# control-toolbox/CTDirect.jl

Hardware: AMD Instinct MI355X
Metric: NLP callback evals/s (constraints+sparse Jac), N-step Goddard, 1/2/4/8 GPU (higher is better)
Workload: dtype f64

## Files before the change

### ctdirect.jl_amd/_lib.py

```python
import ctypes as C
import os
import subprocess

_HERE = os.path.dirname(os.path.abspath(__file__))
LIB_PATH = os.environ.get("CTD_LIB_PATH") or os.path.join(_HERE, "libctdirect_hip.so")
CSRC = os.path.join(_HERE, "csrc")

CTD_OK, CTD_EINVAL, CTD_EGRID, CTD_ESCHEME, CTD_EPATTERN, CTD_EPROBLEM, CTD_ENODEVICE, CTD_EHIP, CTD_ENOMEM, CTD_ERCCL = range(10)


class ctd_desc(C.Structure):
    _fields_ = [("problem", C.c_int32), ("scheme", C.c_int32), ("pattern_mode", C.c_int32), ("device", C.c_int32),
                ("grid_size", C.c_int64), ("time_grid", C.POINTER(C.c_double)), ("time_grid_len", C.c_int64),
                ("step_begin", C.c_int64), ("step_end", C.c_int64), ("stream", C.c_void_p),
                ("stream_mode", C.c_int32), ("control_steps", C.c_int32), ("value_order", C.c_int32), ("reserved0", C.c_int32)]


class ctd_init(C.Structure):
    _fields_ = [("use_problem_default", C.c_int32), ("state", C.POINTER(C.c_double)),
                ("control", C.POINTER(C.c_double)), ("variable", C.POINTER(C.c_double)),
                ("n_samples", C.c_int64), ("t_samples", C.POINTER(C.c_double)),
                ("state_samples", C.POINTER(C.c_double)), ("control_samples", C.POINTER(C.c_double))]


class ctd_ocp_def(C.Structure):
    _fields_ = [("name", C.c_char_p), ("n", C.c_int32), ("m", C.c_int32), ("nv", C.c_int32), ("npath", C.c_int32),
                ("nbc", C.c_int32), ("it0", C.c_int32), ("itf", C.c_int32), ("t0", C.c_double), ("tf", C.c_double),
                ("maximize", C.c_int32), ("reserved", C.c_int32), ("dynamics", C.POINTER(C.c_char_p)),
                ("lagrange", C.c_char_p), ("mayer", C.c_char_p), ("path", C.POINTER(C.c_char_p)),
                ("boundary", C.POINTER(C.c_char_p)), ("constants", C.c_char_p)] + \
               [(k, C.POINTER(C.c_double)) for k in ("state_lb", "state_ub", "control_lb", "control_ub", "variable_lb",
                                                     "variable_ub", "path_lb", "path_ub", "boundary_lb", "boundary_ub")]


_dp = C.POINTER(C.c_double)
_ip = C.POINTER(C.c_int64)
_vp = C.c_void_p
SYMBOLS = {
    "ctd_create": (C.c_int32, [C.POINTER(ctd_desc), C.POINTER(_vp)]),
    "ctd_destroy": (C.c_int32, [_vp]),
    "ctd_last_error": (C.c_char_p, [_vp]),
    "ctd_strerror": (C.c_char_p, [C.c_int32]),
    "ctd_host_alloc": (C.c_int32, [C.POINTER(C.c_void_p), C.c_size_t]),
    "ctd_host_free": (C.c_int32, [C.c_void_p]),
    "ctd_sizes": (C.c_int32, [_vp, _ip, _ip, _ip, _ip]),
    "ctd_dims": (C.c_int32, [_vp, _ip]),
    "ctd_time_grid": (C.c_int32, [_vp, _dp, _dp]),
    "ctd_time_grid_at": (C.c_int32, [_vp, _dp, _dp]),
    "ctd_butcher": (C.c_int32, [_vp, _dp, _dp, _dp]),
    "ctd_bounds": (C.c_int32, [_vp, _dp, _dp, _dp, _dp]),
    "ctd_initial_guess": (C.c_int32, [_vp, _dp, C.POINTER(ctd_init)]),
    "ctd_jac_structure": (C.c_int32, [_vp, _ip, _ip]),
    "ctd_jac_csc": (C.c_int32, [_vp, _ip, _ip]),
    "ctd_jac_csr": (C.c_int32, [_vp, _ip, _ip]),
    "ctd_value_order": (C.c_int32, [_vp, C.POINTER(C.c_int32)]),
    "ctd_dropped_nonzeros": (C.c_int32, [_vp, _ip]),
    "ctd_obj": (C.c_int32, [_vp, _dp, _dp]),
    "ctd_grad": (C.c_int32, [_vp, _dp, _dp]),
    "ctd_grad_dev": (C.c_int32, [_vp, _vp, _vp]),
    "ctd_cons": (C.c_int32, [_vp, _dp, _dp]),
    "ctd_jac_coord": (C.c_int32, [_vp, _dp, _dp]),
    "ctd_cons_jac": (C.c_int32, [_vp, _dp, _dp, _dp]),
    "ctd_cons_jac_dev": (C.c_int32, [_vp, _vp, _vp, _vp]),
    "ctd_cons_jac_dev_async": (C.c_int32, [_vp, _vp, _vp, _vp]),
    "ctd_obj_dev": (C.c_int32, [_vp, _vp, _dp]),
    "ctd_obj_dev_async": (C.c_int32, [_vp, _vp, _vp]),
    "ctd_grad_dev_async": (C.c_int32, [_vp, _vp, _vp]),
    "ctd_grad_shard_dev_async": (C.c_int32, [_vp, _vp, _vp]),
    "ctd_sync": (C.c_int32, [_vp]),
    "ctd_set_stream": (C.c_int32, [_vp, _vp]),
    "ctd_shard_info": (C.c_int32, [_vp, _ip]),
    "ctd_time_cons_jac_dev": (C.c_int32, [_vp, _vp, _vp, _vp, C.c_int32, _dp]),
    "ctd_launch_info": (C.c_int32, [_vp, _ip]),
    "ctd_debug_stamps": (C.c_int32, [_vp, _vp, _vp, _vp, C.POINTER(C.c_uint64), C.c_int64]),
    "ctd_register_ocp": (C.c_int32, [C.POINTER(ctd_ocp_def), C.POINTER(C.c_int32)]),
    "ctd_ocp_source": (C.c_int32, [C.c_int32, C.c_char_p, C.c_int64]),
    "ctd_jit_check": (C.c_int32, [C.c_int32, C.c_int32]),
    "ctd_hess_structure": (C.c_int32, [_vp, _ip, _ip]),
    "ctd_hess_csc": (C.c_int32, [_vp, _ip, _ip]),
    "ctd_hess_csr": (C.c_int32, [_vp, _ip, _ip]),
    "ctd_hess_coord": (C.c_int32, [_vp, _dp, _dp, C.c_double, _dp]),
    "ctd_hess_coord_dev": (C.c_int32, [_vp, _vp, _vp, C.c_double, _vp]),
    "ctd_hess_coord_dev_async": (C.c_int32, [_vp, _vp, _vp, C.c_double, _vp]),
    "ctd_time_hess_dev": (C.c_int32, [_vp, _vp, _vp, C.c_double, _vp, C.c_int32, _dp]),
    "ctd_hess_launch_info": (C.c_int32, [_vp, _ip]),
    "ctd_hess_kernel_info": (C.c_int32, [_vp, _ip]),
    "ctd_hess_shard_info": (C.c_int32, [_vp, _ip]),
    "ctd_hess_debug_stamps": (C.c_int32, [_vp, _vp, _vp, C.c_double, _vp, C.POINTER(C.c_uint64), C.c_int64]),
    "ctd_eval_all_dev_async": (C.c_int32, [_vp, _vp, _vp, C.c_double, _vp, _vp, _vp, _vp, _vp]),
    "ctd_cons_jac_batch_dev_async": (C.c_int32, [_vp, C.c_int32, _vp, C.c_int64, _vp, C.c_int64, _vp, C.c_int64]),
    "ctd_obj_batch_dev_async": (C.c_int32, [_vp, C.c_int32, _vp, C.c_int64, _vp]),
    "ctd_grad_batch_dev_async": (C.c_int32, [_vp, C.c_int32, _vp, C.c_int64, _vp, C.c_int64]),
    "ctd_jprod": (C.c_int32, [_vp, _dp, _dp, _dp]),
    "ctd_jtprod": (C.c_int32, [_vp, _dp, _dp, _dp]),
    "ctd_jprod_dev_async": (C.c_int32, [_vp, _vp, _vp, _vp]),
    "ctd_jtprod_dev_async": (C.c_int32, [_vp, _vp, _vp, _vp]),
    "ctd_hprod": (C.c_int32, [_vp, _dp, _dp, C.c_double, _dp, _dp]),
    "ctd_hprod_dev_async": (C.c_int32, [_vp, _vp, _vp, C.c_double, _vp, _vp]),
    "ctd_kktprod": (C.c_int32, [_vp, _dp, _dp, C.c_double, _dp, _dp, _dp, _dp, _dp, _dp]),
    "ctd_kktprod_dev_async": (C.c_int32, [_vp, _vp, _vp, C.c_double, _vp, _vp, _vp, _vp, _vp, _vp]),
    "ctd_hdiag": (C.c_int32, [_vp, _dp, _dp, C.c_double, _dp]),
    "ctd_hdiag_dev_async": (C.c_int32, [_vp, _vp, _vp, C.c_double, _vp]),
    "ctd_jsq_rows": (C.c_int32, [_vp, _dp, _dp, _dp]),
    "ctd_jsq_rows_dev_async": (C.c_int32, [_vp, _vp, _vp, _vp]),
    "ctd_jsq_cols": (C.c_int32, [_vp, _dp, _dp, _dp]),
    "ctd_jsq_cols_dev_async": (C.c_int32, [_vp, _vp, _vp, _vp]),
    "ctd_jprod_shard_dev_async": (C.c_int32, [_vp, _vp, _vp, _vp]),
    "ctd_jtprod_shard_dev_async": (C.c_int32, [_vp, _vp, _vp, _vp]),
    "ctd_hprod_shard_dev_async": (C.c_int32, [_vp, _vp, _vp, C.c_double, _vp, _vp]),
    "ctd_kktprod_shard_dev_async": (C.c_int32, [_vp, _vp, _vp, C.c_double, _vp, _vp, _vp, _vp, _vp, _vp]),
    "ctd_hess_coord_batch_dev_async": (C.c_int32, [_vp, C.c_int32, _vp, C.c_int64, _vp, C.c_int64, C.c_double, _vp, C.c_int64]),
    "ctd_create_sharded": (C.c_int32, [C.POINTER(ctd_desc), C.POINTER(C.c_int32), C.c_int32, C.POINTER(_vp)]),
    "ctd_sharded_destroy": (C.c_int32, [_vp]),
    "ctd_sharded_last_error": (C.c_char_p, [_vp]),
    "ctd_sharded_handle": (C.c_int32, [_vp, C.c_int32, C.POINTER(_vp)]),
    "ctd_sharded_shard_info": (C.c_int32, [_vp, C.c_int32, _ip]),
    "ctd_cons_jac_sharded_dev_async": (C.c_int32, [_vp, C.POINTER(_vp), C.POINTER(_vp), C.POINTER(_vp), C.c_int32, C.c_int32]),
    "ctd_sharded_sync": (C.c_int32, [_vp]),
    "ctd_dev_alloc": (C.c_int32, [C.c_int32, C.c_size_t, C.POINTER(_vp)]),
    "ctd_dev_free": (C.c_int32, [C.c_int32, _vp]),
    "ctd_dev_copy": (C.c_int32, [C.c_int32, _vp, _vp, C.c_size_t, C.c_int32]),
    "ctd_set_x_shards": (C.c_int32, [_vp, C.c_int32, _ip, C.POINTER(_vp), C.c_int32]),
    "ctd_ipc_export": (C.c_int32, [C.c_int32, _vp, _vp, _ip]),
    "ctd_ipc_open": (C.c_int32, [C.c_int32, _vp, C.POINTER(_vp)]),
    "ctd_ipc_close": (C.c_int32, [C.c_int32, _vp]),
    "ctd_ipc_probe": (C.c_int32, [C.c_int32, _vp, C.c_size_t]),
    "ctd_stitch_c": (C.c_int32, [_vp, _vp, C.c_int32, C.c_int32, _vp]),
    "ctd_shard_steps": (C.c_int32, [C.c_int64, C.c_int32, C.c_int32, _ip, _ip]),
}


def build(jobs=8):
    subprocess.check_call(["make", "-C", CSRC, "-s", f"-j{jobs}"])
    return LIB_PATH


_lib = None


def lib():
    global _lib
    if _lib is None:
        if not os.path.exists(LIB_PATH):
            raise ImportError(
                f"{LIB_PATH} is missing: the HIP extension has not been built (run `python -c 'import "
                "__graft_entry__ as g; g.build()'` or `make -C ctdirect.jl_amd/csrc`). There is no fallback path.")
        try:
# ... 13 lines not shown
```

### ctdirect.jl_amd/csrc/ctd_engine.hip

```cpp
#include <hip/hip_runtime.h>
#include <hip/hiprtc.h>
#include <dlfcn.h>

#include <cstdio>
#include <functional>
#include <map>
#include <mutex>
#include <cstdlib>
#include <cstring>
#include <memory>
#include <new>
#include <string>
#include <vector>

#include "../../include/ctdirect_hip.h"
#include "ctd_host.hpp"
#include "ctd_kernels.hpp"
#include "ctd_hess_kernels.hpp"
#include "ctd_hess_step.hpp"
#include "ctd_iter_kernels.hpp"
#include "ctd_prod_kernels.hpp"
#include "ctd_hprod_kernels.hpp"
#include "ctd_kkt_kernels.hpp"
#include "ctd_diag_kernels.hpp"
#include "ctd_jit.hpp"

using namespace ctd;

namespace ctd {
#define CTD_EXTERN_ALL(ID, P) \
    CTD_EXTERN_LAUNCHERS(P) CTD_EXTERN_HESS(P) CTD_EXTERN_HESS_STEP(P) CTD_EXTERN_ITER(P) CTD_EXTERN_PROD(P) CTD_EXTERN_HPROD(P) CTD_EXTERN_KKT(P) CTD_EXTERN_DIAG(P)
CTD_REGISTRY(CTD_EXTERN_ALL)
}

template <class T = double> struct DevBuf {
    T* p = nullptr;
    int64_t cap = 0;
    DevBuf() = default;
    DevBuf(const DevBuf&) = delete;
    DevBuf& operator=(const DevBuf&) = delete;
    ~DevBuf() { release(); }
    void release() { if (p) (void)hipFree(p); p = nullptr; cap = 0; }
    hipError_t ensure(int64_t n) {
        if (p && n <= cap) return hipSuccess;
        release();
        const hipError_t e = hipMalloc((void**)&p, sizeof(T) * (size_t)(n > 1 ? n : 1));
        if (e == hipSuccess) cap = n; else p = nullptr;
        return e;
    }
    int32_t grow(ctd_handle* h, int64_t need, const char* fn);
};

enum JitFamily { JIT_FIRST, JIT_BATCH, JIT_PROD, JIT_HPROD, JIT_HESS, JIT_PROD_SHARD, JIT_HPROD_SHARD, JIT_KKT, JIT_KKT_SHARD, JIT_DIAG, kJitFamilies };
struct JitModule {
    hipModule_t mod = nullptr;
    hipFunction_t f[5] = {};
};

struct ctd_handle {
    Model model;
    int device = -1;
    hipStream_t stream = nullptr;
    bool own_stream = false;
    int64_t step_begin = 0, step_end = 0;
    int tile = 0, block = 256;
    int lean_ok = 1;
    KParams kp;
    size_t lds_bytes = 0;
    int grid = 0;
    DevBuf<double> d_tau;
    DevBuf<uint32_t> d_tmpl, d_vtmpl;
    DevBuf<uint16_t> d_pos;
    DevBuf<int64_t> d_edge_idx;
    DevBuf<uint32_t> d_edge_code;
    DevBuf<> d_x, d_c, d_vals;
    DevBuf<> d_partial;
    DevBuf<> d_obj;
    DevBuf<> d_g;
    DevBuf<> d_gpartial;
    int obj_blocks = 0;
    hipEvent_t ev0 = nullptr, ev1 = nullptr;
    const RtOcp* rt = nullptr;
    JitModule jit[kJitFamilies];
    bool hess_ready = false;
    HParams hp;
    int hess_tile = 0;
    size_t hess_lds_bytes = 0;
    DevBuf<uint32_t> d_htptr, d_hterms, d_hvptr, d_hvterms, d_heptr, d_hevptr, d_heterms;
    DevBuf<int64_t> d_hedge_idx;
    DevBuf<double> d_hpair_c;
    DevBuf<uint32_t> d_hcpos, d_hzpos;
    DevBuf<int32_t> d_hssrc, d_hschunk;
    DevBuf<double> d_hsck;
    bool hess_step = false;
    SParams sp{};
    HParams hp_step{};
    size_t hess_step_lds = 0;
    DevBuf<uint32_t> d_htasks, d_hptasks, d_hbtasks;
    DevBuf<> d_hpartials, d_y, d_hvals;
    DevBuf<XHalo> d_halo;
    XHalo halo_host{};
    DevBuf<> d_stitch_send, d_stitch_recv;
    int64_t hpart_member = 0;
    double out_mb = 0.0;
    DevBuf<> d_ppartial, d_pdir, d_pout;
    DevBuf<> d_hppartial;
    DevBuf<> d_kktpartial, d_kdy, d_ksx, d_ksc, d_krc;
    DevBuf<> d_hdpartial, d_jcpartial;
    std::string err;
};

constexpr double kWtMB = 64.0;
constexpr double kHessWtMB = 16.0;

static thread_local std::string g_create_err;

static int32_t fail(ctd_handle* h, int32_t code, const std::string& msg) {
    if (h) h->err = msg; else g_create_err = msg;
    return code;
}

#define HIP_TRY(h, expr)                                                                          \
    do {                                                                                          \
        hipError_t e_ = (expr);                                                                   \
        if (e_ != hipSuccess)                                                                     \
            return fail(h, CTD_EHIP, std::string(#expr) + ": " + hipGetErrorString(e_));          \
    } while (0)

struct DeviceGuard {
    int prev = -1;
    bool switched = false;
    hipError_t err = hipSuccess;
    DeviceGuard() = default;
    explicit DeviceGuard(int dev) { (void)bind(dev); }
    hipError_t bind(int dev) {
        err = hipGetDevice(&prev);
        if (err == hipSuccess && prev != dev) { err = hipSetDevice(dev); switched = (err == hipSuccess); }
        return err;
    }
    ~DeviceGuard() { if (switched) (void)hipSetDevice(prev); }
    DeviceGuard(const DeviceGuard&) = delete;
    DeviceGuard& operator=(const DeviceGuard&) = delete;
};

struct OnDevice {
    DeviceGuard dg;
    int32_t st = CTD_OK;
    explicit OnDevice(ctd_handle* h, const char* fn = nullptr) {
        if (!h) st = CTD_EINVAL;
        else if (h->device < 0)
            st = fail(h, CTD_ENODEVICE, std::string(fn ? fn : "") + (fn ? ": " : "") +
                                            "compute call on a host-only handle (device = -1); there is no CPU fallback");
        else if (dg.bind(h->device) != hipSuccess) st = fail(h, CTD_EHIP, std::string("dg_.err: ") + hipGetErrorString(dg.err));
    }
};

template <class T> int32_t DevBuf<T>::grow(ctd_handle* h, int64_t need, const char* fn) {
    if (need <= cap && p) return CTD_OK;
    hipStreamCaptureStatus cs = hipStreamCaptureStatusNone;
    if (hipStreamIsCapturing(h->stream, &cs) == hipSuccess && cs != hipStreamCaptureStatusNone)
        return fail(h, CTD_EINVAL, std::string(fn) + ": this batch needs larger partial-sum buffers, which cannot be allocated while the "
                                   "stream is capturing; make one call with the same batch size before the capture");
    (void)hipGetLastError();
    HIP_TRY(h, hipStreamSynchronize(h->stream));
    HIP_TRY(h, ensure(need));
    return CTD_OK;
}

template <class T> static hipError_t upload(DevBuf<T>& dst, const std::vector<T>& src) {
    dst.release();
    if (src.empty()) return hipSuccess;
    const hipError_t e = dst.ensure((int64_t)src.size());
    if (e != hipSuccess) return e;
    return hipMemcpy(dst.p, src.data(), src.size() * sizeof(T), hipMemcpyHostToDevice);
}

static int env_int(const char* name, int dflt) {
    const char* s = std::getenv(name);
    return (s && *s) ? std::atoi(s) : dflt;
}

static void destroy_handle(ctd_handle* h) {
    DeviceGuard dg;
    if (h->device >= 0) {
        (void)dg.bind(h->device);
        (void)hipStreamSynchronize(h->stream);
        if (h->ev0) (void)hipEventDestroy(h->ev0);
        if (h->ev1) (void)hipEventDestroy(h->ev1);
        if (h->own_stream && h->stream) (void)hipStreamDestroy(h->stream);
        for (JitModule& m : h->jit)
            if (m.mod) (void)hipModuleUnload(m.mod);
    }
    delete h;
}

namespace {
std::string jit_include_dir() {
    const char* env = std::getenv("CTD_JIT_INCLUDE");
    if (env && *env) return env;
    Dl_info info;
    if (dladdr((const void*)&destroy_handle, &info) && info.dli_fname) {
        std::string path(info.dli_fname);
        const size_t slash = path.find_last_of('/');
        return (slash == std::string::npos ? std::string(".") : path.substr(0, slash)) + "/csrc";
    }
    return "csrc";
}

std::mutex g_jit_mu;
std::map<std::string, std::pair<std::string, std::vector<std::string>>> g_jit_cache;

int32_t jit_compile(const RtOcp& ro, const char* header, const std::vector<std::string>& exprs, const char* fp_contract,
                    std::string& code, std::vector<std::string>& lowered, std::string& err) {
    std::string key = ro.name + "|" + std::to_string((size_t)&ro) + "|" + header;
    for (const std::string& e : exprs) key += "|" + e;
    std::vector<std::string> extra;
    if (const char* ex = std::getenv("CTD_JIT_EXTRA")) {
        std::string cur;
        for (const char* c = ex;; ++c) {
            if (*c == ' ' || *c == 0) { if (!cur.empty()) extra.push_back(cur); cur.clear(); if (*c == 0) break; }
            else cur += *c;
        }
        key += std::string("|") + ex;
    }
    {
        std::lock_guard<std::mutex> lk(g_jit_mu);
        auto it = g_jit_cache.find(key);
        if (it != g_jit_cache.end()) { code = it->second.first; lowered = it->second.second; return CTD_OK; }
    }
    const std::string src = std::string("#include \"") + header + "\"\n" + ro.functor_src;
    hiprtcProgram prog = nullptr;
    if (hiprtcCreateProgram(&prog, src.c_str(), "ctd_user_ocp.hip", 0, nullptr, nullptr) != HIPRTC_SUCCESS) {
        err = "hiprtcCreateProgram failed";
        return CTD_EHIP;
    }
    for (const std::string& e : exprs) (void)hiprtcAddNameExpression(prog, e.c_str());
    const std::string inc = "-I" + jit_include_dir();
    const std::string fpc = std::string("-ffp-contract=") + fp_contract;
    std::vector<const char*> opts = {"--offload-arch=gfx950", "-O3", "-std=c++17", fpc.c_str(), inc.c_str()};
    for (const std::string& e : extra) opts.push_back(e.c_str());
    const hiprtcResult rc = hiprtcCompileProgram(prog, (int)opts.size(), opts.data());
    if (rc != HIPRTC_SUCCESS) {
        size_t ls = 0;
        (void)hiprtcGetProgramLogSize(prog, &ls);
        std::string log(ls, '\0');
        if (ls) (void)hiprtcGetProgramLog(prog, &log[0]);
        err = "run-time compilation of OCP '" + ro.name + "' failed: " + log.substr(0, 4000);
        (void)hiprtcDestroyProgram(&prog);
        return CTD_EHIP;
    }
    lowered.clear();
    for (const std::string& e : exprs) {
        const char* ln = nullptr;
        if (hiprtcGetLoweredName(prog, e.c_str(), &ln) != HIPRTC_SUCCESS || !ln) { err = "no lowered name for " + e; (void)hiprtcDestroyProgram(&prog); return CTD_EHIP; }
        lowered.emplace_back(ln);
    }
    size_t cs = 0;
    (void)hiprtcGetCodeSize(prog, &cs);
    code.assign(cs, '\0');
    (void)hiprtcGetCode(prog, &code[0]);
    (void)hiprtcDestroyProgram(&prog);
    std::lock_guard<std::mutex> lk(g_jit_mu);
    g_jit_cache[key] = {code, lowered};
    return CTD_OK;
}
// ... 195 lines not shown
    }
    const bool long_mid = mo.L.sc == SC_MIDPOINT && mo.L.cs == 1;
    if (desc->device >= 0 && !h->rt && env_int("CTD_TILE", 0) <= 0 && mo.nch_dyn <= 1 && (mo.L.sc == SC_IRK || long_mid) && h->tile >= 16) {
        DeviceGuard dgq(desc->device);
        if (dgq.err == hipSuccess) {
            auto resident = [&](int tile, size_t& lds) {
                KParams kq;
                mo.fill_kparams(kq, h->step_begin, h->step_end, tile);
                lds = (size_t)lds_doubles(kq) * sizeof(double);
                int r = 0;
                for_problem(mo.problem, [&](auto tag) { r = occupancy_cons_jac<typename decltype(tag)::type>(kq, h->block, lds); });
                (void)hipGetLastError();
                return r;
            };
            size_t l0 = 0;
            const int r0 = resident(h->tile, l0);
            const int64_t ns = h->step_end - h->step_begin, cap = 256 * (int64_t)r0;
            if (r0 > 0 && (ns + h->tile - 1) / h->tile >= env_int("CTD_LONG_GRID_ROUNDS", 8) * cap && maxb >= 512 && env_int("CTD_BLOCK", 0) <= 0 &&
                env_int("CTD_LONG_GRID", 1)) {
                int tbest = h->tile;
                for (int tt = h->tile + 1; tt <= 256; ++tt) {
                    KParams kq;
                    mo.fill_kparams(kq, h->step_begin, h->step_end, tt);
                    if ((size_t)lds_doubles(kq) * sizeof(double) > (long_mid ? 74u : 64u) * 1024) break;
                    tbest = tt;
                }
                if (tbest > h->tile) {
                    h->tile = tbest;
                    h->block = 512;
                    mo.fill_kparams(h->kp, h->step_begin, h->step_end, h->tile);
                    h->lds_bytes = (size_t)lds_doubles(h->kp) * sizeof(double);
                }
            } else if (mo.L.sc == SC_IRK && r0 > 0 && (ns + h->tile - 1) / h->tile > cap) {
                int tmax = 48;
                for (; tmax > h->tile; --tmax) { size_t l = 0; if (resident(tmax, l) >= r0 && l <= lds_cap) break; }
                const int64_t rounds = (ns + (int64_t)tmax * cap - 1) / ((int64_t)tmax * cap);
                const int64_t tb = (ns + rounds * cap - 1) / (rounds * cap);
                if (tb > h->tile && tb <= tmax) {
                    h->tile = (int)tb;
                    mo.fill_kparams(h->kp, h->step_begin, h->step_end, h->tile);
                    h->lds_bytes = (size_t)lds_doubles(h->kp) * sizeof(double);
                }
            }
        }
    }
    h->grid = h->kp.ntiles + h->kp.has_edge;
    h->kp.debug_stop = debug_stop;
    h->out_mb = 8.0 * ((double)(h->step_end - h->step_begin) * (mo.L.cb + mo.Lseg + (double)mo.L.nv * mo.vr)) / 1.0e6;
    h->kp.wt_store = h->out_mb <= kWtMB ? 1 : 0;
    h->device = desc->device;
    if (h->device >= 0) {
        int ndev = 0;
        if (hipGetDeviceCount(&ndev) != hipSuccess || h->device >= ndev)
            return fail(nullptr, CTD_ENODEVICE, "ctd_create: HIP device not available");
        ctd_handle* hp = h.get();
        if (h->lds_bytes > 160 * 1024) return fail(nullptr, CTD_EINVAL, "ctd_create: tile does not fit the 160 KiB LDS");
        DeviceGuard dg_(hp->device); HIP_TRY(nullptr, dg_.err);
        if (desc->stream_mode == CTD_STREAM_GIVEN) { hp->stream = (hipStream_t)desc->stream; hp->own_stream = false; }
        else { HIP_TRY(nullptr, hipStreamCreateWithFlags(&hp->stream, hipStreamNonBlocking)); hp->own_stream = true; }
        HIP_TRY(nullptr, upload(hp->d_tau, mo.tau));
        HIP_TRY(nullptr, upload(hp->d_tmpl, mo.tmpl));
        HIP_TRY(nullptr, upload(hp->d_vtmpl, mo.vtmpl));
        HIP_TRY(nullptr, upload(hp->d_edge_idx, mo.edge_idx));
        HIP_TRY(nullptr, upload(hp->d_edge_code, mo.edge_code));
        hp->kp.tau = hp->d_tau.p;
        hp->kp.tmpl = hp->d_tmpl.p;
        hp->kp.vtmpl = hp->d_vtmpl.p;
        {
            const int S = mo.L.s, r_dyn = S * mo.nch_dyn, r_path = mo.nch_path;
            int lgT = 0;
            while ((1 << lgT) < hp->tile) ++lgT;
            const int leadbase = (((r_dyn + r_path) << lgT) + 63) & ~63;
            const int early_lanes = mo.n_early + mo.c_early + mo.L.nv * mo.vr_early;
            if (env_int("CTD_EARLY", 0) && mo.n_early > 0 && !hp->rt && mo.fused && hp->tile <= 32 && leadbase + 64 <= hp->block && early_lanes <= 64 &&
                mo.n_late > 0 && mo.n_late <= hp->block) {
                HIP_TRY(nullptr, upload(hp->d_pos, mo.pos_order));
                hp->kp.pos = hp->d_pos.p;
                hp->kp.n_late = mo.n_late; hp->kp.n_early = mo.n_early; hp->kp.c_early = mo.c_early; hp->kp.vr_early = mo.vr_early;
                hp->kp.div_late = make_fastdiv((uint32_t)mo.n_late);
            }
        }
        hp->kp.edge_idx = hp->d_edge_idx.p;
        hp->kp.edge_code = hp->d_edge_code.p;
        hp->obj_blocks = 256;
        HIP_TRY(nullptr, hp->d_partial.ensure(hp->obj_blocks));
        HIP_TRY(nullptr, hp->d_obj.ensure(1));
        HIP_TRY(nullptr, hipEventCreate(&hp->ev0));
        HIP_TRY(nullptr, hipEventCreate(&hp->ev1));
        if (hp->rt) {
            if (hp->lds_bytes > 64 * 1024) return fail(nullptr, CTD_EINVAL, "ctd_create: one step of this run-time OCP does not fit 64 KiB of LDS");
            const int32_t jst = jit_load(hp, JIT_FIRST);
            if (jst) return jst;
        }
        {
            const bool direct = mo.fused && mo.L.sc != SC_TRAPEZE;
            const int mt = env_int("CTD_MULTI_TILE", 0);
            if (!direct && mt > 0 && kMultiTileLoop && !hp->rt) {
                int per_cu = mt > 1 ? mt : 0, cus = 256;
                if (hipDeviceGetAttribute(&cus, hipDeviceAttributeMultiprocessorCount, hp->device) != hipSuccess) cus = 256;
                if (per_cu == 0) {
                    if (hp->rt) {
                        if (hipModuleOccupancyMaxActiveBlocksPerMultiprocessor(&per_cu, hp->jit[JIT_FIRST].f[0], hp->block, hp->lds_bytes) != hipSuccess) per_cu = 0;
                    } else {
                        for_problem(mo.problem, [&](auto tag) {
                            using P = typename decltype(tag)::type;
                            per_cu = occupancy_cons_jac<P>(hp->kp, hp->block, hp->lds_bytes);
                        });
                    }
                }
                const int64_t cap = (int64_t)per_cu * cus - hp->kp.has_edge;
                if (cap > 0 && hp->kp.ntiles > cap) {
                    hp->kp.wg_stride = (int)cap;
                    hp->grid = hp->kp.wg_stride + hp->kp.has_edge;
                }
            }
        }
    }
    *out = h.release();
    return CTD_OK;
}

int32_t ctd_register_ocp(const ctd_ocp_def* def, int32_t* problem_id) {
    if (!def || !problem_id) return fail(nullptr, CTD_EINVAL, "ctd_register_ocp: null argument");
    std::string err;
    int id = -1;
    const int st = register_runtime_ocp(def, &id, err);
    if (st) return fail(nullptr, st, "ctd_register_ocp: " + err);
    *problem_id = id;
    return CTD_OK;
}

int32_t ctd_ocp_source(int32_t problem_id, char* buf, int64_t cap) {
    const RtOcp* ro = runtime_ocp(problem_id);
    if (!ro) return fail(nullptr, CTD_EINVAL, "ctd_ocp_source: not a run-time problem id");
    const int64_t need = (int64_t)ro->functor_src.size() + 1;
    if (!buf || cap < need)
        return fail(nullptr, CTD_EINVAL, "ctd_ocp_source: buffer too small, needs " + std::to_string(need) + " bytes");
    std::memcpy(buf, ro->functor_src.c_str(), (size_t)need);
    return CTD_OK;
}

int32_t ctd_jit_check(int32_t problem_id, int32_t scheme) {
    const RtOcp* ro = runtime_ocp(problem_id);
    if (!ro) return fail(nullptr, CTD_EPROBLEM, "ctd_jit_check: not a run-time problem id");
    if (scheme < 0 || scheme > 8) return fail(nullptr, CTD_ESCHEME, "Unknown discretization method");
    const int sc = scheme == 0 ? SC_TRAPEZE : ((scheme == 1 || scheme >= 7) ? SC_MIDPOINT : SC_IRK);
    int s = (scheme < 2 || scheme >= 7) ? 0 : (scheme <= 4 ? scheme - 1 : scheme - 3);
    if (scheme == 1) s = env_int("CTD_JIT_CHECK_CS", 0);
    std::string code, err;
    std::vector<std::string> names;
    int32_t st = jit_compile(*ro, "ctd_kernels.hpp", jit_first_exprs(sc, s), "off", code, names, err);
    if (st == CTD_OK) st = jit_compile(*ro, "ctd_hess_kernels.hpp", jit_hess_exprs(sc, s), "fast", code, names, err);
    if (st) return fail(nullptr, st, err);
    return CTD_OK;
}

int32_t ctd_destroy(ctd_handle* h) {
    if (!h) return CTD_EINVAL;
    destroy_handle(h);
    return CTD_OK;
}

int32_t ctd_sizes(const ctd_handle* h, int64_t* nvar, int64_t* ncon, int64_t* nnzj, int64_t* nnzh) {
    if (!h) return CTD_EINVAL;
    if (nvar) *nvar = h->model.L.nvar;
    if (ncon) *ncon = h->model.L.ncon;
// ... 243 lines not shown
    const int64_t np = own + mytail;
    stitch_pack_kernel<<<(unsigned)((np + 255) / 256), 256, 0, h->stream>>>(c_dev, h->d_stitch_send.p, h->step_begin * L.cb, own, N * L.cb, mytail);
    HIP_TRY(h, hipGetLastError());
    const int32_t st = check(g_nccl_allgather(h->d_stitch_send.p, h->d_stitch_recv.p, (size_t)smax, kNcclDouble, nccl_comm, h->stream), "ncclAllGather");
    if (st) return st;
    stitch_unpack_kernel<<<(unsigned)((L.ncon + 255) / 256), 256, 0, h->stream>>>(h->d_stitch_recv.p, c_dev, L.ncon, N, L.cb, G, smax);
    HIP_TRY(h, hipGetLastError());
    return CTD_OK;
}

int32_t ctd_ipc_export(int32_t device, const void* dev_ptr, void* handle64, int64_t* offset) {
    if (!dev_ptr || !handle64 || !offset) return CTD_EINVAL;
    static_assert(sizeof(hipIpcMemHandle_t) == 64, "CTD_IPC_HANDLE_BYTES");
    DeviceGuard dg(device);
    hipError_t e = dg.err;
    hipDeviceptr_t base = nullptr;
    size_t size = 0;
    if (e == hipSuccess) e = hipMemGetAddressRange(&base, &size, (hipDeviceptr_t)dev_ptr);
    hipIpcMemHandle_t hd;
    if (e == hipSuccess) e = hipIpcGetMemHandle(&hd, (void*)base);
    if (e != hipSuccess) { g_create_err = std::string("ctd_ipc_export: ") + hipGetErrorString(e); (void)hipGetLastError(); return CTD_EHIP; }
    std::memcpy(handle64, &hd, sizeof(hd));
    *offset = (int64_t)((const char*)dev_ptr - (const char*)base);
    return CTD_OK;
}
int32_t ctd_ipc_open(int32_t device, const void* handle64, void** base) {
    if (!handle64 || !base) return CTD_EINVAL;
    *base = nullptr;
    DeviceGuard dg(device);
    hipError_t e = dg.err;
    hipIpcMemHandle_t hd;
    std::memcpy(&hd, handle64, sizeof(hd));
    if (e == hipSuccess) e = hipIpcOpenMemHandle(base, hd, hipIpcMemLazyEnablePeerAccess);
    if (e != hipSuccess) { g_create_err = std::string("ctd_ipc_open: ") + hipGetErrorString(e); (void)hipGetLastError(); return CTD_ERCCL; }
    return CTD_OK;
}
int32_t ctd_ipc_probe(int32_t device, const void* ptr, size_t bytes) {
    if (!ptr || bytes == 0 || bytes > 64) return CTD_EINVAL;
    DeviceGuard dg(device);
    hipError_t e = dg.err;
    void* tmp = nullptr;
    if (e == hipSuccess) e = hipMalloc(&tmp, 64);
    if (e == hipSuccess) e = hipMemcpy(tmp, ptr, bytes, hipMemcpyDeviceToDevice);
    if (e == hipSuccess) e = hipDeviceSynchronize();
    if (tmp) (void)hipFree(tmp);
    if (e != hipSuccess) { g_create_err = std::string("ctd_ipc_probe: ") + hipGetErrorString(e); (void)hipGetLastError(); return CTD_ERCCL; }
    return CTD_OK;
}
int32_t ctd_ipc_close(int32_t device, void* base) {
    if (!base) return CTD_OK;
    DeviceGuard dg(device);
    return (dg.err == hipSuccess && hipIpcCloseMemHandle(base) == hipSuccess) ? CTD_OK : CTD_EHIP;
}

int32_t ctd_launch_info(const ctd_handle* h, int64_t* o) {
    if (!h || !o) return CTD_EINVAL;
    o[0] = h->grid; o[1] = h->block; o[2] = (int64_t)h->lds_bytes; o[3] = h->tile; o[4] = h->model.Lseg;
    o[5] = (int64_t)h->model.edge_idx.size();
    o[6] = (h->model.fused && h->model.L.sc != SC_TRAPEZE) ? 1 : 0;
    o[7] = 0;
    if (h->device >= 0) {
        DeviceGuard dg(h->device);
        int per_cu = 0;
        if (dg.err == hipSuccess) {
            if (h->rt) { if (hipModuleOccupancyMaxActiveBlocksPerMultiprocessor(&per_cu, h->jit[JIT_FIRST].f[0], h->block, h->lds_bytes) != hipSuccess) per_cu = 0; }
            else for_problem(h->model.problem, [&](auto tag) {
                using P = typename decltype(tag)::type;
                per_cu = occupancy_cons_jac<P>(h->kp, h->block, h->lds_bytes);
            });
        }
        (void)hipGetLastError();
        o[7] = per_cu;
    }
    return CTD_OK;
}


struct Batch {
    int32_t n;
    int64_t ldx, ldy, ldc, ldv, ldg, ldh;
};

static int32_t enqueue_cons_jac(ctd_handle* h, const double* x_dev, double* c_dev, double* vals_dev, hipEvent_t te0 = nullptr,
                                hipEvent_t te1 = nullptr, const Batch* bt = nullptr) {
    const OnDevice on(h);
    if (on.st) return on.st;
    if (!x_dev) return fail(h, CTD_EINVAL, "x is null");
    KParams kp = h->kp;
    kp.c = c_dev;
    kp.vals = vals_dev;
    hipError_t e = hipErrorInvalidValue;
    if (bt) {
        BatchLd bl{bt->ldx, bt->ldc, bt->ldv};
        kp.wt_store = h->out_mb * bt->n <= kWtMB ? 1 : 0;
        if (h->rt) {
            if (const int32_t jst = jit_load(h, JIT_BATCH)) return jst;
            void* args[] = {&kp, &x_dev, &bl};
            e = jit_launch(h->jit[JIT_BATCH].f[0], h->grid, h->block, h->lds_bytes, h->stream, args, nullptr, nullptr, bt->n);
        }
        for_problem(h->model.problem, [&](auto tag) {
            using P = typename decltype(tag)::type;
            e = launch_cons_jac_batch<P>(kp, x_dev, bl, h->grid, h->block, h->lds_bytes, h->stream, bt->n);
        });
        if (e != hipSuccess) return fail(h, CTD_EHIP, std::string("kernel launch: ") + hipGetErrorString(e));
        return CTD_OK;
    }
    if (h->rt) {
        void* args[] = {&kp, &x_dev};
        e = jit_launch(h->jit[JIT_FIRST].f[0], h->grid, h->block, h->lds_bytes, h->stream, args, te0, te1);
    }
    for_problem(h->model.problem, [&](auto tag) {
        using P = typename decltype(tag)::type;
        e = launch_cons_jac<P>(kp, x_dev, h->grid, h->block, h->lds_bytes, h->stream, te0, te1, h->lean_ok);
    });
    if (e != hipSuccess) return fail(h, CTD_EHIP, std::string("kernel launch: ") + hipGetErrorString(e));
    return CTD_OK;
}

int32_t ctd_cons_jac_dev_async(ctd_handle* h, const double* x_dev, double* c_dev, double* vals_dev) {
    return enqueue_cons_jac(h, x_dev, c_dev, vals_dev);
}

int32_t ctd_set_stream(ctd_handle* h, void* stream) {
    if (!h) return CTD_EINVAL;
    if (h->device < 0) return fail(h, CTD_ENODEVICE, "host-only handle");
    if (h->own_stream && h->stream) { (void)hipStreamSynchronize(h->stream); (void)hipStreamDestroy(h->stream); }
    h->stream = (hipStream_t)stream;
    h->own_stream = false;
    return CTD_OK;
}

int32_t ctd_sync(ctd_handle* h) {
    if (!h) return CTD_EINVAL;
    if (h->device < 0) return fail(h, CTD_ENODEVICE, "host-only handle");
    HIP_TRY(h, hipStreamSynchronize(h->stream));
    return CTD_OK;
}

int32_t ctd_cons_jac_dev(ctd_handle* h, const double* x_dev, double* c_dev, double* vals_dev) {
    int32_t st = enqueue_cons_jac(h, x_dev, c_dev, vals_dev);
    if (st) return st;
    return ctd_sync(h);
}

static int32_t host_cons_jac(ctd_handle* h, const double* x, double* c, double* vals) {
    const OnDevice on(h);
    if (on.st) return on.st;
    if (!x) return fail(h, CTD_EINVAL, "x is null");
    const Model& mo = h->model;
    return host_call(h, {{x, h->d_x, mo.L.nvar}},
                     [&] { return enqueue_cons_jac(h, h->d_x.p, c ? h->d_c.p : nullptr, vals ? h->d_vals.p : nullptr); },
                     {{c, h->d_c, mo.L.ncon}, {vals, h->d_vals, mo.nnzj}});
}

int32_t ctd_host_alloc(void** ptr, size_t bytes) {
    if (!ptr) return CTD_EINVAL;
    *ptr = nullptr;
    const hipError_t e = hipHostMalloc(ptr, bytes ? bytes : 8, hipHostMallocDefault);
    if (e != hipSuccess) { g_create_err = std::string("ctd_host_alloc: ") + hipGetErrorString(e); return CTD_EHIP; }
    return CTD_OK;
}
int32_t ctd_host_free(void* ptr) {
    if (!ptr) return CTD_OK;
    return hipHostFree(ptr) == hipSuccess ? CTD_OK : CTD_EHIP;
}

int32_t ctd_cons(ctd_handle* h, const double* x, double* c) {
    if (h && !c) return fail(h, CTD_EINVAL, "c is null");
    return host_cons_jac(h, x, c, nullptr);
}
int32_t ctd_jac_coord(ctd_handle* h, const double* x, double* vals) {
    if (h && !vals) return fail(h, CTD_EINVAL, "vals is null");
    return host_cons_jac(h, x, nullptr, vals);
}
int32_t ctd_cons_jac(ctd_handle* h, const double* x, double* c, double* vals) {
    if (h && (!c || !vals)) return fail(h, CTD_EINVAL, "c or vals is null");
    return host_cons_jac(h, x, c, vals);
}

static int fill_obj_params(ctd_handle* h, double* f_dev, ObjParams& op);

static int32_t enqueue_obj(ctd_handle* h, const double* x_dev, double* f_dev, const Batch* bt = nullptr) {
    const OnDevice on(h);
    if (on.st) return on.st;
    if (!x_dev || !f_dev) return fail(h, CTD_EINVAL, "null argument");
    const Layout& L = h->model.L;
    ObjParams op;
    const int blocks = fill_obj_params(h, f_dev, op);
    const bool lagrange = h->model.info.lagrange;
    const int nb = bt ? bt->n : 1;
    if (bt) {
        const int32_t st = h->d_partial.grow(h, (int64_t)nb * (blocks > 0 ? blocks : 1), "ctd_obj_batch_dev_async");
        if (st) return st;
        op.partial = h->d_partial.p;
        op.ldx = bt->ldx;
    }
    hipError_t e = hipErrorInvalidValue;
    if (h->rt) {
        void* args[] = {&op, &x_dev};
        e = lagrange ? jit_launch(h->jit[JIT_FIRST].f[1], blocks, 256, 0, h->stream, args, nullptr, nullptr, nb) : hipSuccess;
        if (e == hipSuccess) e = jit_launch(h->jit[JIT_FIRST].f[2], 1, 64, 0, h->stream, args, nullptr, nullptr, nb);
    }
    for_problem(h->model.problem, [&](auto tag) {
// ... 1107 lines not shown
```

### ctdirect.jl_amd/csrc/ctd_host.cpp

```cpp
#include "ctd_host.hpp"
#include "ctd_kernel_body.hpp"
#include "ctd_hess_body.hpp"
#include "ctd_jit.hpp"

#include <algorithm>
#include <cmath>
#include <cstdlib>
#include <cstring>
#include <map>
#include <set>

namespace ctd {

enum { ST_OK = 0, ST_EINVAL = 1, ST_EGRID = 2, ST_ESCHEME = 3, ST_EPATTERN = 4, ST_EPROBLEM = 5 };

static void set_butcher(Layout& L, int s) {
    for (double& x : L.a) x = 0.0;
    for (int i = 0; i < 3; ++i) L.b[i] = L.c[i] = 0.0;
    const double r3 = std::sqrt(3.0), r15 = std::sqrt(15.0);
    if (s == 1) {
        L.a[0] = 0.5; L.b[0] = 1.0; L.c[0] = 0.5;
    } else if (s == 2) {
        L.a[0] = 0.25;            L.a[1] = 0.25 - r3 / 6;
        L.a[3] = 0.25 + r3 / 6;   L.a[4] = 0.25;
// ... 792 lines not shown
            if (chk > mo.reg_first && chk < mo.reg_last - 1 && !same(chk)) { err = "Jacobian pattern is not step-periodic by rows"; return ST_EPATTERN; }
        if ((need & 2) && mo.HH == 0) { err = "internal: row template needs the next step's record but the tile has no halo"; return ST_EPATTERN; }
        mo.tmpl = c1;
        mo.cp_tmpl = rp1;
        mo.Lseg = (int)c1.size();
    }
    std::vector<int64_t> cols;
    const int64_t head_rows = mo.reg_first * L.cb;
    mo.cp_head.assign(head_rows + 1, 0);
    int64_t nz = 0;
    for (int64_t r = 0; r < head_rows; ++r) { mo.cp_head[r] = nz; mo.gen_row(r, cols); nz += (int64_t)cols.size(); }
    mo.cp_head[head_rows] = nz;
    mo.seg_base = nz;
    nz += (mo.reg_last - mo.reg_first) * (int64_t)mo.Lseg;
    const int64_t tail0 = mo.reg_last * L.cb, tail_rows = L.ncon - tail0;
    mo.cp_tail.assign(tail_rows + 1, 0);
    for (int64_t rr = 0; rr < tail_rows; ++rr) { mo.cp_tail[rr] = nz; mo.gen_row(tail0 + rr, cols); nz += (int64_t)cols.size(); }
    mo.cp_tail[tail_rows] = nz;
    mo.nnzj = nz;
    struct Raw { int64_t idx; Model::Entry e; };
    std::vector<Raw> first, last;
    std::set<int64_t> needrec;
    needrec.insert(0);
    needrec.insert(N - 1);
    auto scan_row = [&](int64_t r, std::vector<Raw>& dst) {
        mo.gen_row(r, cols);
        const int64_t base = mo.row_start(r);
        for (size_t t = 0; t < cols.size(); ++t) {
            Model::Entry e = mo.classify(r, cols[t]);
            if (e.kind == 0) {
                if (!e.cconst) needrec.insert(e.cstep);
                if (e.di != 0) needrec.insert(e.dstep);
            }
            dst.push_back(Raw{base + (int64_t)t, e});
        }
    };
    mo.head_ptr.assign(mo.reg_first + 1, 0);
    for (int64_t r = 0; r < head_rows; ++r) {
        if (r % L.cb == 0) mo.head_ptr[r / L.cb] = (int)first.size();
        scan_row(r, first);
    }
    mo.head_ptr[mo.reg_first] = (int)first.size();
    for (int64_t r = tail0; r < L.ncon; ++r) scan_row(r, last);
    if ((int)needrec.size() > kMaxEdgeSlots) { err = "internal: too many edge records"; return ST_EPATTERN; }
    std::map<int64_t, int> slot_of;
    mo.n_edge_slots = 0;
    for (int64_t s : needrec) { slot_of[s] = mo.n_edge_slots; mo.edge_steps[mo.n_edge_slots++] = s; }
    mo.edge_fp = mo.n_edge_slots;
    mo.edge_b = mo.n_edge_slots + 1;
    mo.edge_slot_first = slot_of[0];
    mo.edge_slot_last = slot_of[N - 1];
    mo.edge_idx.clear(); mo.edge_code.clear();
    auto emit = [&](const std::vector<Raw>& src) {
        for (const Raw& r : src) {
            const Model::Entry& e = r.e;
            int crec, drec;
            if (e.kind == 0) {
                drec = (e.di != 0) ? slot_of[e.dstep] : slot_of[0];
                crec = (!e.cconst) ? slot_of[e.cstep] : drec;
            } else {
                crec = drec = (e.kind == 1) ? mo.edge_fp : mo.edge_b;
            }
            mo.edge_idx.push_back(r.idx);
            mo.edge_code.push_back(pack_code(e.di, e.ci, e.beta, drec, crec));
        }
    };
    emit(first);
    mo.edge_split = (int)mo.edge_idx.size();
    for (int q = 0; q < L.p; ++q) {
        mo.edge_idx.push_back(kEdgeCBit | (N * L.cb + q));
        mo.edge_code.push_back(pack_code(mo.R.oR + q, C_ONE, 0, mo.edge_fp, mo.edge_fp));
    }
    for (int r = 0; r < L.bc; ++r) {
        mo.edge_idx.push_back(kEdgeCBit | (N * L.cb + L.p + r));
        mo.edge_code.push_back(pack_code(mo.R.oBval + r, C_ONE, 0, mo.edge_b, mo.edge_b));
    }
    mo.edge_split2 = (int)mo.edge_idx.size();
    emit(last);
    mo.pos_order.clear();
    mo.n_late = mo.Lseg; mo.n_early = mo.c_early = mo.vr_early = 0;
    return ST_OK;
}

static void count_dropped(Model& mo) {
    const Layout& L = mo.L;
    const int64_t N = L.N;
    mo.dropped = 0;
    if (mo.pattern_mode == 0 && L.sc == SC_TRAPEZE && L.nv > 0 && (L.free_time || mo.dyn_v))
        mo.dropped = N * (int64_t)L.n * L.nv;
    if (L.euler == 2 && L.p > 0 && L.m > 0 && mo.pattern_mode == 0) {
        int64_t pairs = 0;
        for (int q = 0; q < L.p; ++q)
            for (int c = 0; c < L.m; ++c) pairs += (mo.dep_g.size() > (size_t)q && (mo.dep_g[q] >> (L.n + c) & 1u)) ? 1 : 0;
        mo.dropped += (N - 1) * pairs;
    }
}

int default_tile(const Model& mo, int64_t nsteps) {
    const Layout& L = mo.L;
    const int64_t per_step = (int64_t)(L.blk + mo.R.stride + 1) * 8;
    const int64_t fit = (60 * 1024) / per_step - mo.HL - mo.HH;
    const int64_t cap = (L.sc == SC_IRK) ? 32 : 64;
    int64_t T = 1;
    while (T * 2 <= fit && T * 2 <= cap) T *= 2;
    const bool wide = mo.nch_dyn > 1;
    const bool multi_u = wide && L.sc == SC_MIDPOINT && L.cs > 1;
    if (wide) {
        const int pts = L.sc == SC_IRK ? L.s : 1;
        const int64_t lane_cap = L.sc == SC_IRK ? 64 / (pts + 1) : (multi_u ? 48 : 24);
        const double out_bytes = 8.0 * (double)(mo.Lseg + L.cb + (int64_t)L.nv * mo.vr);
        T = std::max<int64_t>(4, std::min<int64_t>(lane_cap, (int64_t)std::lround(131072.0 / std::max(out_bytes, 1.0))));
        if (multi_u) T = lane_cap;
        for (; T > 4; --T) {
            KParams kp;
            mo.fill_kparams(kp, 0, std::min<int64_t>(L.N, T * 4), (int)T);
            if (wgs_per_cu(lds_doubles(kp) * 8) >= (multi_u ? 2 : 3)) break;
        }
        if (multi_u) {
            const int64_t ns = nsteps > 0 ? nsteps : L.N, rounds = (ns + T * 512 - 1) / (T * 512);
            T = std::max<int64_t>(4, std::min<int64_t>(T, (ns + rounds * 512 - 1) / (rounds * 512)));
        }
    }
    if (nsteps <= 0) nsteps = L.N;
    if ((nsteps + T - 1) / T < 480) T = std::max<int64_t>(4, std::min<int64_t>(T, (nsteps + 479) / 480));
    if (!wide) {
        const int64_t T1 = (nsteps + 511) / 512;
        if (T1 > T && (T1 + mo.HL + mo.HH + 1) * per_step <= (mo.fused ? 80 : 40) * 1024) T = T1;
    }
    return (int)T;
}

void Model::fill_kparams(KParams& kp, int64_t step_begin, int64_t step_end, int tile) const {
    std::memset(&kp, 0, sizeof(kp));
    kp.L = L;
    kp.R = R;
    kp.T = tile;
    kp.HL = HL; kp.HH = HH;
    kp.step_begin = step_begin; kp.step_end = step_end;
    kp.ntiles = (int)((step_end - step_begin + tile - 1) / tile);
    kp.Lseg = Lseg; kp.vr = vr;
    kp.div_cb = make_fastdiv((uint32_t)L.cb);
    kp.div_Lseg = make_fastdiv((uint32_t)(Lseg > 0 ? Lseg : 1));
    kp.div_vr = make_fastdiv((uint32_t)(vr > 0 ? vr : 1));
    kp.div_blk = make_fastdiv((uint32_t)(L.blk > 0 ? L.blk : 1));
    kp.seg_base = seg_base; kp.reg_first = reg_first; kp.reg_last = reg_last;
    for (int k = 0; k < kMaxNV; ++k) kp.vcol_base[k] = vcol_base[k];
    const bool owns_last = step_end == L.N;
    kp.edge_begin = head_ptr[std::min<int64_t>(step_begin, reg_first)];
    kp.edge_end = head_ptr[std::min<int64_t>(step_end, reg_first)];
    kp.edge2_begin = edge_split;
    kp.edge2_end = owns_last ? (int)edge_idx.size() : edge_split2;
    {
        const int nedge = (kp.edge_end - kp.edge_begin) + (kp.edge2_end - kp.edge2_begin);
        int E = nedge > 0 ? 1 : 0;
        if (nedge > 1024) E = std::min(16, (nedge + 511) / 512);
        if (const char* e = std::getenv("CTD_EDGE_BLOCKS")) { const int v = std::atoi(e); if (v >= 1 && nedge > 0) E = std::min(v, 64); }
        kp.has_edge = E;
    }
    kp.n_edge_slots = n_edge_slots;
    kp.edge_fp = edge_fp; kp.edge_b = edge_b;
    kp.edge_slot_first = edge_slot_first; kp.edge_slot_last = edge_slot_last;
    for (int k = 0; k < kMaxEdgeSlots; ++k) kp.edge_steps[k] = edge_steps[k];
    kp.n_late = Lseg; kp.n_early = kp.c_early = kp.vr_early = 0;
    kp.div_late = make_fastdiv((uint32_t)(Lseg > 0 ? Lseg : 1));
    kp.stage_codes = (Lseg + L.nv * vr <= kMaxStagedCodes) ? 1 : 0;
    if (kp.stage_codes) {
        const int with = wgs_per_cu(lds_doubles(kp) * 8);
        kp.stage_codes = 0;
        const int without = wgs_per_cu(lds_doubles(kp) * 8);
        kp.stage_codes = (without > with && with < 4) ? 0 : 1;
    }
}

int build_model(const HostDesc& d, Model& mo, std::string& err) {
    mo.problem = d.problem;
    mo.pattern_mode = d.pattern_mode;
    if (d.pattern_mode < 0 || d.pattern_mode > 2) { err = "unknown pattern mode"; return ST_EPATTERN; }
    bool found = for_problem(d.problem, [&](auto tag) {
        using P = typename decltype(tag)::type;
        mo.info = P::info();
        mo.dyn_t = P::DYN_T;
        mo.dyn_v = P::DYN_V;
        mo.nch_dyn = Dirs<P>::NCH_DYN;
        mo.nch_path = (P::NPATH > 0) ? Dirs<P>::NCH_PATH : 0;
        mo.fused = Dirs<P>::FUSED;
        mo.H.hk = HessK<P>::value;
        mo.n_f = mo.n_g = -1;
        if (DynNZ<P>::sparse) {
            mo.n_f = DynNZ<P>::nF; mo.n_g = DynNZ<P>::nG;
            mo.map_f.assign(P::NX * P::NX, -1); mo.map_g.assign(P::NX * P::NU, -1);
            for (int r = 0; r < P::NX; ++r) {
                for (int c = 0; c < P::NX; ++c) mo.map_f[r * P::NX + c] = DynNZ<P>::fx(r, c);
                for (int c = 0; c < P::NU; ++c) mo.map_g[r * P::NU + c] = DynNZ<P>::gu(r, c);
            }
        }
    });
    if (!found) {
        const RtOcp* ro = runtime_ocp(d.problem);
        if (!ro) { err = "problem id not in the compiled registry"; return ST_EPROBLEM; }
        mo.info = ro->info;
        mo.dyn_t = ro->dyn_t;
        mo.dyn_v = ro->dyn_v;
        const int dyn = ro->info.n + ro->info.m + (ro->dyn_t ? 1 : 0) + (ro->dyn_v ? ro->info.nv : 0);
        const int pth = ro->info.n + ro->info.m + (ro->path_t ? 1 : 0) + (ro->path_v ? ro->info.nv : 0);
        mo.nch_dyn = (dyn + ro->dc - 1) / ro->dc;
        mo.nch_path = ro->info.npath > 0 ? (pth + ro->dc - 1) / ro->dc : 0;
        mo.fused = mo.nch_dyn == 1 && (ro->info.npath == 0 || mo.nch_path == 1);
        mo.H.hk = ro->hk;
        mo.n_f = mo.n_g = -1;
        if (ro->dyn_nz.sparse) { mo.n_f = ro->dyn_nz.n_f; mo.n_g = ro->dyn_nz.n_g; mo.map_f = ro->dyn_nz.map_f; mo.map_g = ro->dyn_nz.map_g; }
    }
    if (d.scheme < 0 || d.scheme > 8) { err = "Unknown discretization method"; return ST_ESCHEME; }
    int64_t N = 0;
    int st = build_time(mo, d, N, err);
    if (st) return st;
    st = build_layout(mo, d.scheme, N, d.control_steps, err);
    if (st) return st;
    build_tail_blocks(mo);
    compute_dep_masks(mo);
    if (d.value_order != 0 && d.value_order != 1) { err = "unknown value order (CTD_ORDER_CSC = 0, CTD_ORDER_CSR = 1)"; return ST_EINVAL; }
    mo.order = d.value_order;
    st = mo.order == 1 ? build_tables_csr(mo, err) : build_tables(mo, err);
    if (st) return st;
    count_dropped(mo);
    return build_hess_model(mo, err);
}

}
```

### ctdirect.jl_amd/csrc/ctd_host.hpp

```cpp
#pragma once
#include <cstdint>
#include <string>
#include <vector>

#include "ctd_layout.hpp"
#include "ctd_hess.hpp"
#include "ctd_problems.hpp"

namespace ctd {

struct HostDesc {
    int problem, scheme, pattern_mode;
    int64_t grid_size;
    const double* time_grid;
    int64_t time_grid_len;
    int control_steps = 1;
    int value_order = 0;
};

struct Block { int64_t r0, r1, c0, c1; };

struct HessModel {
    HessRecLayout R;
    int hk = 4;
    bool sym_stage = false;
    int64_t nnzh = 0;
    std::vector<Block> tail;
    int Lseg = 0, HL = 0, HH = 0;
    int64_t seg_base = 0, reg_first = 0, reg_last = 0;
    std::vector<uint32_t> tptr, terms;
    std::vector<int64_t> relrow;
    std::vector<uint32_t> tcode;
    int compact = 0;
    std::vector<uint32_t> cpos, ctptr, zpos;
    std::vector<uint32_t> vptr, vterms;
    int nvv = 0;
    int64_t vv_idx[kMaxNV * (kMaxNV + 1) / 2] = {0};
    std::vector<int64_t> edge_idx;
    std::vector<uint32_t> eptr, evptr, eterms;
    int edge_split = 0;
    std::vector<int> head_ptr;
    int n_edge_slots = 0, edge_fp = 0, edge_b = 0;
    int64_t edge_steps[kMaxHessEdgeSlots] = {0};
    std::vector<uint8_t> need_stage, need_path, need_bnd, need_rk;
    std::vector<uint32_t> tasks, ptasks, btasks;
    std::vector<uint16_t> pairs;
    std::vector<uint16_t> pair_kind;
    std::vector<double> pair_c;
    std::vector<int64_t> cp_head, cp_tmpl, cp_tail;
};

struct Model {
    int problem = 0, pattern_mode = 0;
    int order = 0;
    ProblemInfo info;
    Layout L;
    RecLayout R;
    bool dyn_t = false, dyn_v = false;
    int nch_dyn = 1, nch_path = 0;
    int n_f = -1, n_g = -1;
    std::vector<int> map_f, map_g;
    bool fused = true;
    bool uniform = true;
    std::vector<double> tau;
    double fixed_time(int64_t i) const { return L.free_time ? 0.0 : L.t0 + (tau[i] * (L.tf - L.t0)); }
    void fill_bounds(double* var_l, double* var_u, double* con_l, double* con_u) const;
    std::vector<Block> tail;
    int64_t nnzj = 0;
    int64_t dropped = 0;
    std::vector<uint32_t> tmpl, vtmpl;
    int Lseg = 0, vr = 0;
    int64_t seg_base = 0, reg_first = 0, reg_last = 0;
    int64_t vcol_base[kMaxNV] = {0, 0, 0, 0};
    int HL = 0, HH = 0;
    std::vector<uint16_t> pos_order;
    int n_late = 0, n_early = 0, c_early = 0, vr_early = 0;
    std::vector<int64_t> edge_idx;
    std::vector<uint32_t> edge_code;
    int edge_split = 0, edge_split2 = 0;
    std::vector<int> head_ptr;
    int n_edge_slots = 0, edge_fp = 0, edge_b = 0, edge_slot_first = 0, edge_slot_last = 0;
    int64_t edge_steps[kMaxEdgeSlots] = {0};
    std::vector<int64_t> cp_head, cp_tmpl, cp_tail;

    std::vector<uint32_t> dep_f, dep_g, dep_b;
    bool opt_dep(int64_t row, int64_t col) const;

    struct Entry { int kind; int64_t cstep, dstep; int ci, di, beta; bool cconst; };
    Entry classify(int64_t row, int64_t col) const;
    void step_blocks(int64_t i, std::vector<Block>& out) const;
    void gen_column(int64_t j, std::vector<int64_t>& rows) const;
    void rows_from_blocks(int64_t j, const std::vector<Block>& cand, std::vector<int64_t>& rows) const;
    void gen_vcolumn_piece(int k, int64_t i0, int64_t i1, bool with_tail, std::vector<int64_t>& rows) const;
    int64_t column_start(int64_t j) const;
    void gen_row(int64_t r, std::vector<int64_t>& cols) const;
    int64_t row_start(int64_t r) const;
    int64_t shard_vals_begin(int64_t step_begin) const;
    int64_t shard_vals_end(int64_t step_end) const;
    void fill_kparams(KParams& kp, int64_t step_begin, int64_t step_end, int tile) const;

    HessModel H;
    void hess_step_blocks(int64_t i, std::vector<Block>& out) const;
    void hess_gen_column(int64_t j, std::vector<int64_t>& rows) const;
    int64_t hess_column_start(int64_t j) const;
    void fill_hparams(HParams& hp, int tile, int64_t step_begin = 0, int64_t step_end = 0) const;
};

void compute_dep_masks(Model& m);
int build_hess_model(Model& m, std::string& err);
bool build_hess_step_tables(const Model& m, const short* pairs, int nout, int chunk, std::vector<int32_t>& src, std::vector<int32_t>& chunk_pos);
int default_hess_tile(const Model& m);

int build_model(const HostDesc& d, Model& m, std::string& err);
struct InitSamples { int64_t n = 0; const double* t = nullptr; const double* state = nullptr; const double* control = nullptr; };
void model_initial_guess(const Model& m, double* x0, bool use_problem_default, const double* state, const double* control,
                         const double* variable, const InitSamples& samples = InitSamples{});
int default_tile(const Model& m, int64_t nsteps = 0);

}
```

### ctdirect.jl_amd/csrc/ctd_kernel_body.hpp

```cpp
#pragma once
#include "ctd_layout.hpp"


namespace ctd {

#if defined(CTD_SUBSTAMPS) && defined(__HIP_DEVICE_COMPILE__)
#ifndef CTD_SUB_WAVE0
#define CTD_SUB_WAVE0 0
#endif
#define CTD_SUB(kp, id)                                                                                              \
    do {                                                                                                             \
        __builtin_amdgcn_sched_barrier(0);                                                                           \
        __builtin_amdgcn_s_waitcnt(0);                                                                               \
        if ((kp).stamps && (threadIdx.x & 63) == 0 && threadIdx.x >= 64 * CTD_SUB_WAVE0 && threadIdx.x < 64 * CTD_SUB_WAVE0 + 128) \
            (kp).stamps[(size_t)gridDim.x * 12 + ((size_t)blockIdx.x * 2 + (threadIdx.x >> 6) - CTD_SUB_WAVE0) * 8 + (id)] = clock64(); \
        __builtin_amdgcn_sched_barrier(0);                                                                           \
    } while (0)
#else
#define CTD_SUB(kp, id) do { } while (0)
#endif
#if defined(CTD_SUBSTAMPS_EMIT) && defined(__HIP_DEVICE_COMPILE__)
#define CTD_SUBE(kp, id)                                                                                             \
    do {                                                                                                             \
        __builtin_amdgcn_sched_barrier(0);                                                                           \
// ... 1298 lines not shown
            if (fold_g) {
                const int64_t i = slot_index<LEAN>(kp, cx, k);
                if (i >= 0 && i < kp.L.N) fin_path<P, SC, S>(kp, cx.rec + k * R.stride, slot_tau<LEAN>(kp, cx, k, 0));
            }
        } else {
            CTD_SUB(kp, 1);
            fin_lead<P, SC, S, LEAN>(kp, cx, k);
            CTD_SUB(kp, 4);
        }
    }
    for (int k = tid; k < ns; k += nthr) cx.rec[k * R.stride] = 1.0;
    CTD_SUB(kp, 5);
}

template <class P, int SC, int S>
CTD_HD void phase_fin(const KParams& kp, const BlockCtx& cx, int tid, int nthr) {
    if (Dirs<P>::FUSED) return;
    if (fin_folded<P, SC, S>(cx)) return;
    constexpr RecLayout R = RL<P, SC, S>::R;
    const int ns = cx.nslots;
    constexpr int rows = (SC == SC_IRK && P::NX > 4) ? P::NX : 1;
    const bool split = split_eval<P, SC, S>(cx, nthr);
    const bool esl = edge_sym_layout<P, SC, S>(cx, nthr);
    const int n_stage = esl ? 0 : StagePoints<SC, S>::value * ns * rows, n_lead = split ? 0 : ns, n_path = (P::NPATH > 0 && !split) ? ns : 0;
    const int n_fp = (cx.is_edge && P::NPATH > 0) ? 1 : 0;
    for (int task = tid; task < n_stage + n_lead + n_path + n_fp; task += nthr) {
        int t = task;
        if (t < n_stage) {
            const int k = t % ns, jr = t / ns;
            if (rows > 1) fin_stage_row<P, S>(kp, cx, k, jr / rows, jr % rows);
            else fin_stage<P, SC, S>(kp, cx, k, jr, cx.rec + k * R.stride + R.oEval + jr * R.eval_sz);
            if (split && P::NPATH > 0 && jr == 0) {
                const int64_t i = slot_index(kp, cx, k);
                if (i >= 0 && i < kp.L.N) fin_path<P, SC, S>(kp, cx.rec + k * R.stride, slot_tau(kp, cx, k, 0));
            }
            continue;
        }
        t -= n_stage;
        if (t < n_lead) { fin_lead<P, SC, S>(kp, cx, t); continue; }
        t -= n_lead;
        if (t < n_path) {
            const int64_t i = slot_index(kp, cx, t);
            if (i >= 0 && i < kp.L.N) fin_path<P, SC, S>(kp, cx.rec + t * R.stride, slot_tau(kp, cx, t, 0));
            continue;
        }
        fin_path<P, SC, S>(kp, cx.rec + kp.edge_fp * R.stride, final_tau(kp, cx));
    }
}

template <class P, int SC, int S>
CTD_HD void phase_fin2(const KParams& kp, const BlockCtx& cx, int tid, int nthr) {
    if (SC == SC_TRAPEZE && !cx.is_edge)
        for (int k = tid; k < cx.nslots; k += nthr) fin_trapeze_step<P>(kp, cx, k);
}

CTD_HD double eval_code(int oC, const double* rec_c, const double* rec_d, uint32_t code) {
    const double coef = rec_c[oC + code_ci(code)];
    const double data = rec_d[code_di(code)];
    const int bt = code_beta(code);
    const double beta = bt == 0 ? 0.0 : (bt == 1 ? 1.0 : -1.0);
    return coef * data + beta;
}

CTD_HD int edge_share_begin(const KParams& kp, const BlockCtx& cx, int ntot) {
    const int E = kp.has_edge > 1 ? kp.has_edge : 1, per = (ntot + E - 1) / E;
    const int lo = cx.edge_part * per;
    return lo < ntot ? lo : ntot;
}
CTD_HD int edge_share_end(const KParams& kp, const BlockCtx& cx, int ntot) {
    const int E = kp.has_edge > 1 ? kp.has_edge : 1, per = (ntot + E - 1) / E;
    const int hi = (cx.edge_part + 1) * per;
    return hi < ntot ? hi : ntot;
}

template <class P, int SC, int S> struct EmitN {
    static constexpr int n = P::NX, m = P::NU, nv = P::NV, p = P::NPATH, s = SC == SC_IRK ? S : 0;
    static constexpr int seg = SC == SC_IRK ? n * (2 * n + s * n + nv) + s * n * (n + s * m + s * n + nv) + p * (n + s * m + nv)
                                            : n * (2 * n + 2 * m * (SC == SC_MIDPOINT ? S : 1) + nv) + p * (n + 2 * m + nv);
#ifndef CTD_PRE_MAX
#define CTD_PRE_MAX 1
#endif
    static constexpr int value = (seg + 255) / 256 < 1 ? 1 : ((seg + 255) / 256 > CTD_PRE_MAX ? CTD_PRE_MAX : (seg + 255) / 256);
};
template <class P, int NB = 1, bool LEAN = false>
CTD_HD EmitPreT<NB> emit_prefetch(const KParams& kp, const BlockCtx& cx, int tid, int nthr) {
    EmitPreT<NB> pre;
    pre.b = 0u;
    pre.eidx = 0;
    pre.have = 1;
    pre.kpos = 0; pre.eb = 0u; pre.ek = 0;
#pragma unroll
    for (int q = 0; q < (NB > 1 ? NB - 1 : 1); ++q) pre.more[q] = 0u;
#pragma unroll
    for (int kk = 0; kk < kMaxNV; ++kk) pre.v[kk] = 0u;
    if (cx.is_edge) {
        const int n1 = kp.edge_end - kp.edge_begin, ntot = n1 + (kp.edge2_end - kp.edge2_begin);
        const int w = edge_share_begin(kp, cx, ntot) + tid;
        if (w < edge_share_end(kp, cx, ntot)) {
            const int e = w < n1 ? kp.edge_begin + w : kp.edge2_begin + (w - n1);
            pre.b = kp.edge_code[e];
            pre.eidx = kp.edge_idx[e];
        }
        return pre;
    }
    const int Ls = kp.Lseg;
    pre.kpos = 0; pre.eb = 0u; pre.ek = 0;
    if (!LEAN && kp.n_early > 0) {
        const int q = tid - (int)fast_div((uint32_t)tid, kp.div_late) * kp.n_late;
        pre.kpos = kp.pos[q];
        pre.b = kp.tmpl[pre.kpos];
        const int l = tid & 63;
        if (l < kp.n_early) { pre.ek = kp.pos[kp.n_late + l]; pre.eb = kp.tmpl[pre.ek]; }
        else if (l >= kp.n_early + kp.c_early && l < kp.n_early + kp.c_early + P::NV * kp.vr_early) {
            const int e = l - kp.n_early - kp.c_early, kk = e / kp.vr_early;
            pre.ek = e - kk * kp.vr_early;
            pre.eb = kp.vtmpl[kk * kp.vr + pre.ek];
        }
    } else if (Ls > 0 && Ls <= nthr) {
        const int k = tid - (int)fast_div((uint32_t)tid, kp.div_Lseg) * Ls;
        pre.b = kp.tmpl[k];
    } else if (Ls > nthr) {
        pre.b = kp.tmpl[tid];
        if constexpr (NB > 1) {
#pragma unroll
            for (int q = 0; q < NB - 1; ++q)
                if (tid + (q + 1) * nthr < Ls) pre.more[q] = kp.tmpl[tid + (q + 1) * nthr];
        }
    }
    const int vr = kp.vr;
#pragma unroll
    for (int kk = 0; kk < kMaxNV; ++kk) {
        if (kk < P::NV && vr > 0 && vr <= nthr) {
            const int k = tid - (int)fast_div((uint32_t)tid, kp.div_vr) * vr;
            pre.v[kk] = kp.vtmpl[kk * vr + k];
        }
    }
    return pre;
}

template <class P, int SC, int S, int NB = 1, bool B = false, bool LEAN = false>
CTD_HD void phase_emit_impl(const KParams& kp, const BlockCtx& cx, int tid, int nthr, const EmitPreT<NB> pre_v, const bool hp,
                            const BatchLd bl = BatchLd{}) {
    const Layout& L = kp.L;
    constexpr RecLayout R = RL<P, SC, S>::R;
    const EmitPreT<NB>* pre_ = &pre_v;
    if (cx.is_edge) {
        const int n1 = kp.edge_end - kp.edge_begin, nall = n1 + (kp.edge2_end - kp.edge2_begin);
        const int wlo = edge_share_begin(kp, cx, nall), ntot = edge_share_end(kp, cx, nall);
        for (int w0 = wlo + tid; w0 < ntot; w0 += 4 * nthr) {
            uint32_t code[4];
            int64_t idx[4];
#pragma unroll
            for (int u = 0; u < 4; ++u) {
                const int w = w0 + u * nthr;
                const int e = w < n1 ? kp.edge_begin + w : kp.edge2_begin + (w - n1);
                const bool have = hp && w == wlo + tid;
                code[u] = have ? pre_->b : (w < ntot ? kp.edge_code[e] : 0u);
                idx[u] = have ? pre_->eidx : (w < ntot ? kp.edge_idx[e] : 0);
            }
#pragma unroll
            for (int u = 0; u < 4; ++u) {
                if (w0 + u * nthr >= ntot) break;
                const double val = eval_code(R.oC, cx.rec + code_crec(code[u]) * R.stride, cx.rec + code_drec_raw(code[u]) * R.stride, code[u]);
                if (idx[u] & kEdgeCBit) { if (kp.c) out_c<B>(kp, bl)[idx[u] & ~kEdgeCBit] = val; }
                else if (kp.vals) out_vals<B>(kp, bl)[idx[u]] = val;
            }
        }
        return;
    }
    const int nsteps = (int)(cx.b - cx.a);
    const int slot0 = (int)(cx.a - cx.lo);
    CTD_SUBE(kp, 0);
    const int stride = R.stride;
    if (kp.c) {
        using V = LV<P, SC, S, LEAN>;
        const int cb = V::cb(kp);
        double* out = out_c<B>(kp, bl) + cx.a * (int64_t)cb;
        const int par = (int)V::div_cb(kp, (uint32_t)nthr);
        if (par >= 1) {
            if (tid < par * cb) {
                const int g = (int)V::div_cb(kp, (uint32_t)tid), r = tid - g * cb;
                const double* src = cx.rec + (slot0 + g) * stride + R.oR + r;
                if (LEAN || r >= kp.c_early)
                    for (int s = g; s < nsteps; s += par, src += par * stride) emit_store(&out[s * cb + r], *src, kp.wt_store);
            }
        } else {
            for (int r = tid; r < cb; r += nthr) {
                const double* src = cx.rec + slot0 * stride + R.oR + r;
                for (int s = 0; s < nsteps; ++s, src += stride) emit_store(&out[s * cb + r], *src, kp.wt_store);
            }
        }
    }
    CTD_SUBE(kp, 1);
    if (!kp.vals) return;
    {
        const int64_t ra = cx.a > kp.reg_first ? cx.a : kp.reg_first;
        const int64_t rb = cx.b < kp.reg_last ? cx.b : kp.reg_last;
        if (rb > ra) {
            const int Ls = kp.Lseg;
            const int nreg = (int)(rb - ra);
            double* out = out_vals<B>(kp, bl) + kp.seg_base + (ra - kp.reg_first) * (int64_t)Ls;
            const int sl0 = (int)(ra - cx.lo);
            const bool late_only = !LEAN && kp.n_early > 0;
            const int Lw = late_only ? kp.n_late : Ls;
            const int par = (int)fast_div((uint32_t)nthr, late_only ? kp.div_late : kp.div_Lseg);
            if (par >= 1) {
                if (tid < par * Lw) {
                    const int g = (int)fast_div((uint32_t)tid, late_only ? kp.div_late : kp.div_Lseg);
                    const int k = late_only ? (hp ? pre_->kpos : (int)kp.pos[tid - g * Lw]) : tid - g * Ls;
                    const uint32_t code = hp ? pre_->b : cx.codes[k];
                    const int bt = code_beta(code);
                    const double beta = bt == 0 ? 0.0 : (bt == 1 ? 1.0 : -1.0);
                    const double* pc = cx.rec + (sl0 - code_crec(code)) * stride + R.oC + code_ci(code);
                    const double* pd = cx.rec + (sl0 - code_drec(code)) * stride + code_di(code);
                    const int last = nreg - 1;
                    for (int s0 = g; s0 < nreg; s0 += 4 * par) {
                        double a[4], b[4];
#pragma unroll
                        for (int u = 0; u < 4; ++u) {
                            const int s = s0 + u * par < last ? s0 + u * par : last;
                            a[u] = pc[s * stride];
                            b[u] = pd[s * stride];
                        }
#pragma unroll
                        for (int u = 0; u < 4; ++u) {
                            const int s = s0 + u * par;
                            if (s < nreg) emit_store(&out[s * Ls + k], a[u] * b[u] + beta, kp.wt_store);
                        }
                    }
                }
            } else {
                uint32_t code = (hp && tid < Ls) ? pre_->b : (tid < Ls ? cx.codes[tid] : 0u);
                int q = 0;
                for (int k = tid; k < Ls; k += nthr, ++q) {
                    uint32_t nxt = 0u;
                    bool have = false;
                    if constexpr (NB > 1) {
                        if (hp && q < NB - 1) {
                            have = true;
#pragma unroll
                            for (int e = 0; e < NB - 1; ++e)
                                if (e == q) nxt = pre_->more[e];
                        }
                    }
                    if (!have) nxt = k + nthr < Ls ? cx.codes[k + nthr] : 0u;
                    const int bt = code_beta(code);
                    const double beta = bt == 0 ? 0.0 : (bt == 1 ? 1.0 : -1.0);
                    const double* pc = cx.rec + (sl0 - code_crec(code)) * stride + R.oC + code_ci(code);
                    const double* pd = cx.rec + (sl0 - code_drec(code)) * stride + code_di(code);
                    const int last = nreg - 1;
                    for (int s0 = 0; s0 < nreg; s0 += 4) {
                        double a[4], b[4];
#pragma unroll
                        for (int u = 0; u < 4; ++u) {
                            const int s = s0 + u < last ? s0 + u : last;
                            a[u] = pc[s * stride];
                            b[u] = pd[s * stride];
                        }
#pragma unroll
                        for (int u = 0; u < 4; ++u)
                            if (s0 + u < nreg) emit_store(&out[(s0 + u) * Ls + k], a[u] * b[u] + beta, kp.wt_store);
                    }
                    code = nxt;
                }
            }
        }
    }
    CTD_SUBE(kp, 2);
    if (kp.vr > 0) {
        const int vr = kp.vr;
        const int par = (int)fast_div((uint32_t)nthr, kp.div_vr);
#pragma unroll
        for (int kk = 0; kk < P::NV; ++kk) {
            double* out = out_vals<B>(kp, bl) + kp.vcol_base[kk] + cx.a * (int64_t)vr;
            const uint32_t* codes = cx.vcodes + kk * vr;
            if (par >= 1) {
                if (tid < par * vr) {
                    const int g = (int)fast_div((uint32_t)tid, kp.div_vr), k = tid - g * vr;
                    const uint32_t code = hp ? pre_->v[kk] : codes[k];
                    const double* pc = cx.rec + (slot0 + g) * stride + R.oC + code_ci(code);
                    const double* pd = cx.rec + (slot0 + g) * stride + code_di(code);
                    const int adv = par * stride;
                    if (LEAN || k >= kp.vr_early)
                        for (int s = g; s < nsteps; s += par, pc += adv, pd += adv) emit_store(&out[s * vr + k], (*pc) * (*pd), kp.wt_store);
                }
            } else {
                for (int k = tid; k < vr; k += nthr) {
                    const uint32_t code = codes[k];
                    const double* pc = cx.rec + slot0 * stride + R.oC + code_ci(code);
                    const double* pd = cx.rec + slot0 * stride + code_di(code);
                    for (int s = 0; s < nsteps; ++s, pc += stride, pd += stride) emit_store(&out[s * vr + k], (*pc) * (*pd), kp.wt_store);
                }
            }
        }
    }
    CTD_SUBE(kp, 3);
}
template <class P, int SC, int S, int NB = 1, bool B = false, bool LEAN = false>
CTD_HD void phase_emit(const KParams& kp, const BlockCtx& cx, int tid, int nthr, const EmitPreT<NB>* pre = nullptr,
                       const BatchLd bl = BatchLd{}) {
    if (pre != nullptr) phase_emit_impl<P, SC, S, NB, B, LEAN>(kp, cx, tid, nthr, *pre, pre->have != 0, bl);
    else phase_emit_impl<P, SC, S, NB, B, LEAN>(kp, cx, tid, nthr, EmitPreT<NB>{}, false, bl);
}

}

#if !defined(__HIPCC_RTC__)
#include "ctd_problems.hpp"
#include "ctd_sym_registry.hpp"
#endif
```

### ctdirect.jl_amd/csrc/ctd_kernels.hpp

```cpp
#pragma once
#if !defined(__HIPCC_RTC__)
#include <hip/hip_runtime.h>
#include <hip/hip_ext.h>
#endif

#include "ctd_kernel_body.hpp"
#if !defined(__HIPCC_RTC__)
#include "ctd_problems.hpp"
#endif

namespace ctd {

#ifndef CTD_MULTI_TILE_LOOP
#define CTD_MULTI_TILE_LOOP 0
#endif
constexpr bool kMultiTileLoop = CTD_MULTI_TILE_LOOP != 0;

template <bool DBG>
__device__ __forceinline__ void ctd_stamp(const KParams& kp, int slot) {
    if constexpr (DBG) {
        if (kp.stamps && threadIdx.x == 0) {
            unsigned long long* p = kp.stamps + ((size_t)blockIdx.x * 6 + slot) * 2;
            p[0] = wall_clock64();
            p[1] = clock64();
        }
    }
}

template <int S, bool LEAN = false>
__device__ __forceinline__ void ctd_pin_kernargs(const KParams& kp, const double* xu) {
#if defined(__HIP_DEVICE_COMPILE__)
    if constexpr (LEAN) {
        asm volatile("" ::"s"(kp.has_edge), "s"(kp.ntiles), "s"(kp.T), "s"(kp.HL), "s"(kp.HH), "s"(kp.step_begin),
                     "s"(kp.step_end), "s"(kp.L.N), "s"(kp.L.v_off), "s"(kp.L.stagewise), "s"(kp.L.euler), "s"(kp.tau), "s"(kp.L.t0),
                     "s"(kp.L.tf), "s"(xu), "s"(blockDim.x));
        asm volatile("" ::"s"(kp.tmpl), "s"(kp.vtmpl), "s"(kp.Lseg), "s"(kp.vr), "s"(kp.div_Lseg.M), "s"(kp.div_vr.M),
                     "s"(kp.div_Lseg.d), "s"(kp.div_vr.d), "s"(kp.seg_base), "s"(kp.reg_first), "s"(kp.reg_last),
                     "s"(kp.vcol_base[0]), "s"(kp.c), "s"(kp.vals));
        return;
    }
    asm volatile("" ::"s"(kp.has_edge), "s"(kp.ntiles), "s"(kp.T), "s"(kp.HL), "s"(kp.HH), "s"(kp.step_begin),
                 "s"(kp.step_end), "s"(kp.L.blk), "s"(kp.L.N), "s"(kp.L.v_off), "s"(kp.L.cu), "s"(kp.L.stagewise), "s"(kp.L.nv),
                 "s"(kp.L.cb), "s"(kp.L.eqs), "s"(kp.L.euler), "s"(kp.tau), "s"(kp.L.t0), "s"(kp.L.tf), "s"(xu), "s"(blockDim.x));
    asm volatile("" ::"s"(kp.tmpl), "s"(kp.vtmpl), "s"(kp.Lseg), "s"(kp.vr), "s"(kp.div_cb.M), "s"(kp.div_Lseg.M), "s"(kp.div_vr.M),
                 "s"(kp.div_cb.d), "s"(kp.div_Lseg.d), "s"(kp.div_vr.d), "s"(kp.seg_base), "s"(kp.reg_first), "s"(kp.reg_last),
                 "s"(kp.vcol_base[0]), "s"(kp.c), "s"(kp.vals), "s"(kp.halo), "s"(kp.pos), "s"(kp.n_early), "s"(kp.n_late));
    if (S >= 1) asm volatile("" ::"s"(kp.L.a[0]), "s"(kp.L.b[0]), "s"(kp.L.c[0]));
    if (S >= 2) asm volatile("" ::"s"(kp.L.a[1]), "s"(kp.L.a[3]), "s"(kp.L.a[4]), "s"(kp.L.b[1]), "s"(kp.L.c[1]));
    if (S >= 3) asm volatile("" ::"s"(kp.L.a[2]), "s"(kp.L.a[5]), "s"(kp.L.a[6]), "s"(kp.L.a[7]), "s"(kp.L.a[8]), "s"(kp.L.b[2]), "s"(kp.L.c[2]));
#endif
}

template <bool LEAN = false>
__device__ __forceinline__ void ctd_pin_emit_kernargs(const KParams& kp) {
#if defined(__HIP_DEVICE_COMPILE__)
    if constexpr (LEAN)
        asm volatile("" ::"s"(kp.c), "s"(kp.vals), "s"(kp.Lseg), "s"(kp.vr), "s"(kp.div_Lseg.M), "s"(kp.div_vr.M),
                     "s"(kp.div_Lseg.d), "s"(kp.div_vr.d), "s"(kp.seg_base), "s"(kp.reg_first), "s"(kp.reg_last),
                     "s"(kp.vcol_base[0]));
    else
        asm volatile("" ::"s"(kp.c), "s"(kp.vals), "s"(kp.L.cb), "s"(kp.Lseg), "s"(kp.vr), "s"(kp.div_cb.M), "s"(kp.div_Lseg.M), "s"(kp.div_vr.M),
                     "s"(kp.div_cb.d), "s"(kp.div_Lseg.d), "s"(kp.div_vr.d), "s"(kp.seg_base), "s"(kp.reg_first), "s"(kp.reg_last),
                     "s"(kp.vcol_base[0]), "s"(kp.n_early), "s"(kp.c_early), "s"(kp.vr_early), "s"(kp.n_late), "s"(kp.div_late.M), "s"(kp.div_late.d));
#endif
}

template <class P, int SC, int S, bool DBG, bool B = false, bool LEAN = false>
__device__ __forceinline__ void cons_jac_body(const KParams& kp, const double* __restrict__ xu, int block, double* ctd_lds,
                                              const BatchLd bl = BatchLd{}) {
    if constexpr (B) xu += batch_member() * bl.ldx;
    ctd_pin_kernargs<SC == SC_IRK ? S : 0, LEAN>(kp, xu);
    ctd_stamp<DBG>(kp, 0);
    if (DBG && kp.debug_stop == 1) return;
    const int tid = (int)threadIdx.x, nthr = (int)blockDim.x;
    if constexpr (DirectTile<P, SC>::value) {
        const BlockCtx cx = make_direct_ctx<LEAN>(kp, block, ctd_lds, xu, LV<P, SC, S, LEAN>::blk(kp), LEAN ? P::NV : -1);
        const EmitPre pre = emit_prefetch<P, 1, LEAN>(kp, cx, tid, nthr);
        ctd_stamp<DBG>(kp, 1);
        phase_eval<P, SC, S, RegEval<P, SC, S>::value, 1, B, LEAN>(kp, cx, tid, nthr, &pre, bl);
        ctd_pin_emit_kernargs<LEAN>(kp);
        __syncthreads();
        ctd_stamp<DBG>(kp, 2);
        ctd_stamp<DBG>(kp, 3);
        if (DBG && kp.debug_stop >= 2 && kp.debug_stop <= 4) return;
        phase_emit<P, SC, S, 1, B, LEAN>(kp, cx, tid, nthr, &pre, bl);
        ctd_stamp<DBG>(kp, 4);
        if (DBG && kp.stamps) {
            __builtin_amdgcn_s_waitcnt(0);
            __syncthreads();
            ctd_stamp<DBG>(kp, 5);
        }
        return;
    }
    BlockCtx cx = make_ctx<LEAN>(kp, block, ctd_lds);
    constexpr int NB = EmitN<P, SC, S>::value;
    EmitPreT<NB> pre = {};
    const bool use_pre = !cx.is_edge && !codes_staged(kp);
    if (use_pre) pre = emit_prefetch<P, NB, LEAN>(kp, cx, tid, nthr);
    phase_load<P, SC, S, true, LEAN>(kp, cx, xu, tid, nthr);
    const int nblk = kp.ntiles + kp.has_edge;
    for (;;) {
        __syncthreads();
        ctd_stamp<DBG>(kp, 1);
        if (DBG && kp.debug_stop == 2) return;
        phase_eval<P, SC, S, false, 1, B, LEAN>(kp, cx, tid, nthr, nullptr, bl);
        ctd_pin_emit_kernargs<LEAN>(kp);
        __syncthreads();
        ctd_stamp<DBG>(kp, 2);
        if (DBG && kp.debug_stop == 3) return;
        if (!Dirs<P>::FUSED && !fin_folded<P, SC, S>(cx)) {
            phase_fin<P, SC, S>(kp, cx, tid, nthr);
            __syncthreads();
        }
        if (SC == SC_TRAPEZE) {
            phase_fin2<P, SC, S>(kp, cx, tid, nthr);
            __syncthreads();
        }
        ctd_stamp<DBG>(kp, 3);
        if (DBG && kp.debug_stop == 4) return;
        block += kp.wg_stride;
        const bool more = kMultiTileLoop && kp.wg_stride > 0 && !cx.is_edge && block < nblk;
        BlockCtx nx = cx;
        TileIn tin{0.0, 0.0, 0.0};
        if (more) {
            nx = make_ctx<LEAN>(kp, block, ctd_lds);
            tin = load_issue<P>(kp, nx, xu, tid, nthr);
        }
        phase_emit_impl<P, SC, S, NB, B, LEAN>(kp, cx, tid, nthr, pre, use_pre, bl);
        ctd_stamp<DBG>(kp, 4);
        if (!more) break;
        load_commit<P, SC, S>(kp, nx, xu, tin, tid, nthr);
        cx = nx;
    }
    if (DBG && kp.stamps) {
        __builtin_amdgcn_s_waitcnt(0);
        __syncthreads();
        ctd_stamp<DBG>(kp, 5);
    }
}

template <class P, int SC, int S> struct MinWaves {
    static constexpr int value = (P::NX <= 12 && !(SC == SC_MIDPOINT && S > 1)) ? 4 : 1;
};

template <class P, int SC, int S, bool DBG, bool LEAN = false>
__global__ void __launch_bounds__(P::MAXB, (MinWaves<P, SC, S>::value)) cons_jac_kernel(const KParams kp, const double* __restrict__ xu) {
    extern __shared__ double ctd_lds[];
    cons_jac_body<P, SC, S, DBG, false, LEAN>(kp, xu, (int)blockIdx.x, ctd_lds);
}
template <class P, int SC, int S>
__global__ void __launch_bounds__(P::MAXB, (MinWaves<P, SC, S>::value)) cons_jac_batch_kernel(const KParams kp, const double* __restrict__ xu,
                                                                                          const BatchLd bl) {
    extern __shared__ double ctd_lds[];
    cons_jac_body<P, SC, S, false, true>(kp, xu, (int)blockIdx.x, ctd_lds, bl);
}

struct ObjParams {
    Layout L;
    const double* tau;
    int64_t unit_begin, unit_end;
    int32_t add_mayer;
    double* partial;
    double* out;
    int32_t nblocks;
    const XHalo* halo;
    XNear near;
    int64_t ldx;
};

template <class P> __device__ double obj_time(const ObjParams& op, const double* v, int64_t i) {
    const double t0 = (P::IT0 >= 0) ? v[P::IT0 >= 0 ? P::IT0 : 0] : op.L.t0;
    const double tf = (P::ITF >= 0) ? v[P::ITF >= 0 ? P::ITF : 0] : op.L.tf;
    const double tau = op.tau ? op.tau[i] : (double)i / (double)op.L.N;
    return t0 + tau * (tf - t0);
}

template <class P, int SC>
__device__ double lagrange_unit(const ObjParams& op, const double* __restrict__ xu, const double* v, int64_t i) {
    constexpr int n = P::NX, m = P::NU;
    const Layout& L = op.L;
    const double* base = xu + i * (int64_t)L.blk;
    const int64_t gn = (i + 1) * (int64_t)L.blk;
    const double* nxt = ((op.halo && i + 1 >= op.unit_end) ? xnear(op.near, xu, gn) : xu) + gn;
    double x[n > 0 ? n : 1], u[m > 0 ? m : 1];
    if (SC == SC_TRAPEZE) {
        double w;
        if (i == 0) w = (obj_time<P>(op, v, 1) - obj_time<P>(op, v, 0)) / 2.0;
        else if (i == L.N) w = (obj_time<P>(op, v, L.N) - obj_time<P>(op, v, L.N - 1)) / 2.0;
        else w = (obj_time<P>(op, v, i + 1) - obj_time<P>(op, v, i - 1)) / 2.0;
        for (int c = 0; c < n; ++c) x[c] = base[c];
        for (int c = 0; c < m; ++c) u[c] = base[n + c];
        return w * P::template lagrange<double>(obj_time<P>(op, v, i), x, u, v);
    }
    const double ti = obj_time<P>(op, v, i), tip1 = obj_time<P>(op, v, i + 1);
    const double h = tip1 - ti;
    if (SC == SC_MIDPOINT) {
        if (L.cs > 1) {
            const double hi = h / (double)L.cs;
            for (int c = 0; c < n; ++c) x[c] = 0.5 * (base[c] + nxt[c]);
            double val = 0.0;
            for (int j = 1; j <= L.cs; ++j) {
                for (int c = 0; c < m; ++c) u[c] = base[n + (j - 1) * m + c];
                const double term = hi * P::template lagrange<double>(ti + ((double)j - 0.5) * hi, x, u, v);
                val = (j == 1) ? term : val + term;
            }
            return val;
        }
        for (int c = 0; c < m; ++c) u[c] = base[n + c];
        if (L.euler == 0) {
            for (int c = 0; c < n; ++c) x[c] = 0.5 * (base[c] + nxt[c]);
            return h * P::template lagrange<double>(0.5 * (ti + tip1), x, u, v);
        }
        for (int c = 0; c < n; ++c) x[c] = (L.euler == 1) ? base[c] : nxt[c];
        return h * P::template lagrange<double>(L.euler == 1 ? ti : tip1, x, u, v);
    }
    const double* K = base + n + L.cu;
    double local = 0.0;
    for (int j = 0; j < L.s; ++j) {
        for (int c = 0; c < n; ++c) {
            double xc = base[c];
            for (int l = 0; l < L.s; ++l) xc = xc + h * L.a[3 * j + l] * K[l * n + c];
            x[c] = xc;
        }
        const double* U = base + n + (L.stagewise ? j * m : 0);
        for (int c = 0; c < m; ++c) u[c] = U[c];
        const double term = L.b[j] * P::template lagrange<double>(ti + L.c[j] * h, x, u, v);
        local = (j == 0) ? term : local + term;
    }
    return h * local;
}

// ... 303 lines not shown
            }
            for (int k = 0; k < nv; ++k) {
                const double dh = FREE ? dtime_of<P>(t1, k) - dtime_of<P>(t0, k) : 0.0;
                gv[k] = gv[k] + dh * sum_bl;
            }
            for (int c = 0; c < n; ++c) g[i * L.blk + c] = gx[c];
            if (!L.stagewise) for (int c = 0; c < m; ++c) g[i * L.blk + n + c] = gu[c];
#pragma unroll
            for (int l = 0; l < S; ++l)
                for (int c = 0; c < n; ++c) g[i * L.blk + n + L.cu + l * n + c] = gK[l][c];
        }
    }
    const int lane = threadIdx.x & 63, wave = threadIdx.x >> 6;
    for (int k = 0; k < nv; ++k) {
        double a = gv[k];
        for (int off = 32; off > 0; off >>= 1) a += __shfl_down(a, off, 64);
        if (lane == 0) wsum[wave][k] = a;
    }
    __syncthreads();
    if (threadIdx.x == 0)
        for (int k = 0; k < nv; ++k) {
            double sacc = 0.0;
            for (int w = 0; w < (int)(blockDim.x >> 6); ++w) sacc += wsum[w][k];
            gp.partial[((size_t)mb * gp.nblocks + block) * kMaxNV + k] = sacc;
        }
}
template <class P, int SC, int S>
__global__ void __launch_bounds__(256) __attribute__((amdgpu_waves_per_eu(2))) grad_units_kernel(const GradParams gp, const double* __restrict__ xu) {
    __shared__ double wsum[4][kMaxNV];
    const int64_t mb = batch_member();
    grad_units_body<P, SC, S>(gp, xu + mb * gp.ldx, (int)blockIdx.x, wsum, mb);
}

template <class P>
__device__ __forceinline__ void grad_finish_body(const GradParams& gp, const double* __restrict__ xu, int64_t mb = 0) {
    if (threadIdx.x >= 64) return;
    constexpr int n = P::NX, nv = P::NV;
    const Layout& L = gp.L;
    const double* part = gp.partial + (size_t)mb * gp.nblocks * kMaxNV;
    double* const g = gp.g + mb * gp.ldg;
    double gvs[nv > 0 ? nv : 1];
    for (int k = 0; k < nv; ++k) {
        double sacc = 0.0;
        for (int b = threadIdx.x; b < gp.nblocks; b += 64) sacc += part[(size_t)b * kMaxNV + k];
        for (int off = 32; off > 0; off >>= 1) sacc += __shfl_down(sacc, off, 64);
        gvs[k] = sacc;
    }
    if (threadIdx.x != 0) return;
    if (P::HAS_MAYER && (gp.owns_first || gp.owns_last)) {
        double x0[n > 0 ? n : 1], xf[n > 0 ? n : 1], v[nv > 0 ? nv : 1], g0x[n > 0 ? n : 1], gfx[n > 0 ? n : 1], gmv[nv > 0 ? nv : 1];
        const double* b0 = grad_block(gp, xu, 0);
        const double* bf = grad_block(gp, xu, L.N);
        for (int c = 0; c < n; ++c) { x0[c] = b0[c]; xf[c] = bf[c]; g0x[c] = 0.0; gfx[c] = 0.0; }
        for (int k = 0; k < nv; ++k) { v[k] = xu[L.v_off + k]; gmv[k] = 0.0; }
        mayer_partials<P, 0>(x0, xf, v, g0x, gfx, gmv);
        for (int c = 0; c < n; ++c) {
            if (gp.owns_first) g[c] += g0x[c];
            if (gp.owns_last) g[L.N * (int64_t)L.blk + c] += gfx[c];
        }
        if (gp.owns_last) for (int k = 0; k < nv; ++k) gvs[k] += gmv[k];
    }
    for (int k = 0; k < nv; ++k) g[L.v_off + k] = gvs[k];
}
template <class P>
__global__ void grad_finish_kernel(const GradParams gp, const double* __restrict__ xu) {
    if (blockIdx.x != 0) return;
    const int64_t mb = batch_member();
    grad_finish_body<P>(gp, xu + mb * gp.ldx, mb);
}

#if !defined(__HIPCC_RTC__)
template <class P>
hipError_t launch_grad(const GradParams& gp, const double* xu, int grid, hipStream_t st, int batch) {
    const dim3 g(grid > 0 ? grid : 1, batch);
    if (grid > 0)
        for_scheme<false>(gp.L, [&](auto t) { grad_units_kernel<P, t.sc, t.s><<<g, 256, 0, st>>>(gp, xu); });
    grad_finish_kernel<P><<<dim3(1, batch), 64, 0, st>>>(gp, xu);
    return hipGetLastError();
}

#endif

#if !defined(__HIPCC_RTC__)
template <class P, int SC, int S, bool DBG, bool LEAN>
hipError_t launch_variant_dbg(const KParams& kp, const double* xu, int grid, int block, size_t lds_bytes, hipStream_t st,
                              hipEvent_t e0, hipEvent_t e1) {
    if (lds_bytes > 64 * 1024) {
        hipError_t e = hipFuncSetAttribute((const void*)cons_jac_kernel<P, SC, S, DBG, LEAN>, hipFuncAttributeMaxDynamicSharedMemorySize,
                                           (int)lds_bytes);
        if (e != hipSuccess) return e;
    }
    if (e0 || e1) hipExtLaunchKernelGGL((cons_jac_kernel<P, SC, S, DBG, LEAN>), dim3(grid), dim3(block), lds_bytes, st, e0, e1, 0, kp, xu);
    else cons_jac_kernel<P, SC, S, DBG, LEAN><<<grid, block, lds_bytes, st>>>(kp, xu);
    return hipGetLastError();
}
template <class P, int SC, int S>
hipError_t launch_variant(const KParams& kp, const double* xu, int grid, int block, size_t lds_bytes, hipStream_t st,
                          hipEvent_t e0, hipEvent_t e1, int lean_ok) {
    const bool dbg = kp.stamps || kp.debug_stop;
    constexpr bool kHasLean = DirectTile<P, SC>::value || SC == SC_IRK;
    if constexpr (kHasLean) {
        if (lean_ok && kp.halo == nullptr && kp.n_early == 0) {
            if (dbg) return launch_variant_dbg<P, SC, S, true, true>(kp, xu, grid, block, lds_bytes, st, e0, e1);
            return launch_variant_dbg<P, SC, S, false, true>(kp, xu, grid, block, lds_bytes, st, e0, e1);
        }
    }
    if (dbg) return launch_variant_dbg<P, SC, S, true, false>(kp, xu, grid, block, lds_bytes, st, e0, e1);
    return launch_variant_dbg<P, SC, S, false, false>(kp, xu, grid, block, lds_bytes, st, e0, e1);
}

template <class P>
hipError_t launch_cons_jac(const KParams& kp, const double* xu, int grid, int block, size_t lds_bytes, hipStream_t st,
                           hipEvent_t e0, hipEvent_t e1, int lean_ok) {
    hipError_t e = hipErrorInvalidValue;
    for_scheme<true>(kp.L, [&](auto t) { e = launch_variant<P, t.sc, t.s>(kp, xu, grid, block, lds_bytes, st, e0, e1, lean_ok); });
    return e;
}

template <class P, int SC, int S>
int occupancy_variant(int block, size_t lds_bytes) {
    int nb = 0;
    if (lds_bytes > 64 * 1024 &&
        hipFuncSetAttribute((const void*)cons_jac_kernel<P, SC, S, false>, hipFuncAttributeMaxDynamicSharedMemorySize, (int)lds_bytes) != hipSuccess)
        return 0;
    if (hipOccupancyMaxActiveBlocksPerMultiprocessor(&nb, cons_jac_kernel<P, SC, S, false>, block, lds_bytes) != hipSuccess) return 0;
    return nb;
}
template <class P, int SC, int S>
hipError_t launch_variant_batch(const KParams& kp, const double* xu, const BatchLd& bl, int grid, int block, size_t lds_bytes, hipStream_t st,
                                int batch) {
    if (lds_bytes > 64 * 1024) {
        hipError_t e = hipFuncSetAttribute((const void*)cons_jac_batch_kernel<P, SC, S>, hipFuncAttributeMaxDynamicSharedMemorySize, (int)lds_bytes);
        if (e != hipSuccess) return e;
    }
    cons_jac_batch_kernel<P, SC, S><<<dim3(grid, batch), block, lds_bytes, st>>>(kp, xu, bl);
    return hipGetLastError();
}
template <class P>
hipError_t launch_cons_jac_batch(const KParams& kp, const double* xu, const BatchLd& bl, int grid, int block, size_t lds_bytes,
                                 hipStream_t st, int batch) {
    hipError_t e = hipErrorInvalidValue;
    for_scheme<true>(kp.L, [&](auto t) { e = launch_variant_batch<P, t.sc, t.s>(kp, xu, bl, grid, block, lds_bytes, st, batch); });
    return e;
}

template <class P>
int occupancy_cons_jac(const KParams& kp, int block, size_t lds_bytes) {
    int nb = 0;
    for_scheme<true>(kp.L, [&](auto t) { nb = occupancy_variant<P, t.sc, t.s>(block, lds_bytes); });
    return nb;
}

template <class P>
hipError_t launch_obj(const ObjParams& op, const double* xu, int grid, int block, hipStream_t st, int batch) {
    const dim3 g(grid > 0 ? grid : 1, batch);
    if (grid > 0)
        for_scheme<false>(op.L, [&](auto t) { obj_partial_kernel<P, t.sc><<<g, block, 0, st>>>(op, xu); });
    obj_finish_kernel<P><<<dim3(1, batch), 64, 0, st>>>(op, xu);
    return hipGetLastError();
}

#define CTD_INSTANTIATE_LAUNCHERS(P)                                                                                       \
    template hipError_t launch_cons_jac<P>(const KParams&, const double*, int, int, size_t, hipStream_t, hipEvent_t, \
                                           hipEvent_t, int);                                                                 \
    template hipError_t launch_cons_jac_batch<P>(const KParams&, const double*, const BatchLd&, int, int, size_t, hipStream_t, int); \
    template hipError_t launch_obj<P>(const ObjParams&, const double*, int, int, hipStream_t, int);                  \
    template int occupancy_cons_jac<P>(const KParams&, int, size_t);                                                 \
    template hipError_t launch_grad<P>(const GradParams&, const double*, int, hipStream_t, int);
#define CTD_EXTERN_LAUNCHERS(P)                                                                                            \
    extern template hipError_t launch_cons_jac<P>(const KParams&, const double*, int, int, size_t, hipStream_t,      \
                                                  hipEvent_t, hipEvent_t, int);                                              \
    extern template hipError_t launch_cons_jac_batch<P>(const KParams&, const double*, const BatchLd&, int, int, size_t, hipStream_t, \
                                                        int);                                                                      \
    extern template hipError_t launch_obj<P>(const ObjParams&, const double*, int, int, hipStream_t, int);          \
    extern template int occupancy_cons_jac<P>(const KParams&, int, size_t);                                         \
    extern template hipError_t launch_grad<P>(const GradParams&, const double*, int, hipStream_t, int);

#endif

}
```

### ctdirect.jl_amd/csrc/ctd_layout.hpp

```cpp
#pragma once
#include "ctd_common.hpp"

namespace ctd {

enum SchemeClass { SC_TRAPEZE = 0, SC_MIDPOINT = 1, SC_IRK = 2 };

constexpr int kMaxNV = 4;
constexpr int kMaxEdgeSlots = 6;

struct Layout {
    int32_t scheme;
    int32_t sc;
    int32_t s;
    int32_t stagewise;
    int32_t n, m, nv, p, bc;
    int32_t cu;
    int32_t blk;
    int32_t eqs;
    int32_t cb;
    int32_t final_control;
    int32_t it0, itf;
    int32_t free_time;
    int64_t N;
    int64_t nvar, ncon;
// ... 105 lines not shown
    return step < cut ? (int)(step / (base + 1)) : (int)(rem + (step - cut) / base);
}
CTD_HD int64_t stitch_src(int64_t r, int64_t N, int cb, int G, int64_t smax) {
    if (r < N * cb) {
        const int64_t step = r / cb;
        const int k = shard_of_step(N, G, step);
        return k * smax + (step - shard_begin(N, G, k)) * cb + (r - step * cb);
    }
    const int64_t last_rows = (N - shard_begin(N, G, G - 1)) * cb;
    return (int64_t)(G - 1) * smax + last_rows + (r - N * cb);
}

CTD_HD const double* xsrc(const XHalo* hl, const double* xu, int64_t g) {
    const int G = hl->G;
    if (g >= hl->vbegin[G]) return xu;
    int k = 0;
    while (k + 1 < G && g >= hl->vbegin[k + 1]) ++k;
    return k == hl->self ? xu : hl->x[k];
}

struct XNear {
    int64_t own_lo, own_hi;
    int64_t prev_lo;
    int64_t last_lo, v_off;
    const double *prev, *next, *first, *last;
};
CTD_HD const double* xnear(const XNear& nr, const double* xu, int64_t g) {
    if ((g >= nr.own_lo && g < nr.own_hi) || g >= nr.v_off) return xu;
    const double* p = g >= nr.own_hi ? (g >= nr.last_lo ? nr.last : nr.next) : (g >= nr.prev_lo ? nr.prev : nr.first);
    return p ? p : xu;
}
inline XNear make_xnear(const XHalo& t, int64_t blk, int64_t N, int64_t v_off) {
    XNear nr{};
    const int G = t.G, me = t.self;
    nr.own_lo = t.vbegin[me]; nr.own_hi = t.vbegin[me + 1];
    nr.prev_lo = nr.own_lo - blk; nr.last_lo = N * blk; nr.v_off = v_off;
    nr.prev = me > 0 ? t.x[me - 1] : nullptr;
    nr.next = me + 1 < G ? t.x[me + 1] : nullptr;
    nr.first = me > 0 ? t.x[0] : nullptr;
    nr.last = me + 1 < G ? t.x[G - 1] : nullptr;
    return nr;
}

struct KParams {
    Layout L;
    RecLayout R;
    const double* tau;
    int32_t T;
    int32_t HL, HH;
    int32_t ntiles;
    int32_t has_edge;
    int32_t xcd_remap;
    int64_t step_begin, step_end;
    const uint32_t* tmpl;
    int32_t Lseg;
    int32_t vr;
    FastDiv div_cb, div_Lseg, div_vr, div_blk;
    int64_t seg_base;
    int64_t reg_first, reg_last;
    const uint32_t* vtmpl;
    int64_t vcol_base[kMaxNV];
    const int64_t* edge_idx;
    const uint32_t* edge_code;
    int32_t edge_begin, edge_end;
    int32_t edge2_begin, edge2_end;
    int32_t n_edge_slots;
    int32_t edge_fp, edge_b;
    int32_t edge_slot_first, edge_slot_last;
    int64_t edge_steps[kMaxEdgeSlots];
    double* c;
    double* vals;
    unsigned long long* stamps;
    int32_t debug_stop;
    int32_t stage_codes;
    const uint16_t* pos;
    int32_t n_late, n_early;
    int32_t c_early, vr_early;
    FastDiv div_late;
    const XHalo* halo;
    XNear near;
    int32_t wg_stride;
    int32_t wt_store;
};
struct BatchLd {
    int64_t ldx, ldc, ldv;
};

}
```

### ctdirect.jl_amd/docp.py

```python
import ctypes as C
from types import SimpleNamespace

import numpy as np

from . import _lib

SCHEMES = {
    "trapeze": 0,
    "midpoint": 1,
    "gauss_legendre_1": 2,
    "gauss_legendre_2_constant_control": 3,
    "gauss_legendre_3_constant_control": 4,
    "gauss_legendre_2": 5,
    "gauss_legendre_3": 6,
    "euler": 7,
    "euler_implicit": 8,
}
SCHEME_ALIASES = {"euler_explicit": "euler", "euler_forward": "euler", "euler_backward": "euler_implicit"}
PROBLEMS = {
    "goddard": 0,
    "goddard_all": 1,
    "double_integrator_path": 2,
    "quadrotor": 3,
    "quadrotor12": 4,
    "stagewise_scalar": 5,
    "estimate_initial_condition": 6,
    "estimate_rotation_rate": 7,
    "least_squares_with_constraint": 8,
    "double_integrator_freet0tf": 9,
}
PATTERN_MODES = {"manual": 0, "reference_manual": 0, "structural": 1, "optimized": 2}
VALUE_ORDERS = {"csc": 0, "csr": 1}


class CTDirectError(RuntimeError):
    def __init__(self, status, message):
        super().__init__(f"[ctd status {status}] {message}")
        self.status = status


def _raise(status, msg):
    if status == _lib.CTD_EGRID:
        raise ValueError(msg)
    raise CTDirectError(status, msg)


def _dp(a):
    return a.ctypes.data_as(C.POINTER(C.c_double)) if a is not None else None


def _ip(a):
    return a.ctypes.data_as(C.POINTER(C.c_int64))


def _host_out(a, n, name):
    if not (isinstance(a, np.ndarray) and a.dtype == np.float64 and a.flags["C_CONTIGUOUS"] and a.flags["WRITEABLE"] and a.size == n):
        raise ValueError(f"{name} must be a writeable C-contiguous float64 NumPy array of {n} entries")
    return a


def _is_tensor(x):
    return hasattr(x, "data_ptr") and hasattr(x, "is_cuda")


def register_ocp(name, *, dynamics, n=None, m=0, nv=0, lagrange=None, mayer=None, path=(), boundary=(), constants=None,
                 t0=0.0, tf=1.0, it0=-1, itf=-1, maximize=False, state_box=None, control_box=None, variable_box=None,
                 path_bounds=None, boundary_bounds=None):
    L = _lib.lib()
    dynamics = list(dynamics)
    n = len(dynamics) if n is None else int(n)
    path, boundary = list(path), list(boundary)
    d = _lib.ctd_ocp_def()
    keep = []

    def strs(items):
        arr = (C.c_char_p * max(len(items), 1))(*[s.encode() for s in items])
        keep.append(arr)
        return C.cast(arr, C.POINTER(C.c_char_p))

    def dbl(seq, dim, fill):
        a = np.full(dim, fill, dtype=np.float64) if seq is None else np.ascontiguousarray(seq, dtype=np.float64)
        if a.size != dim:
            raise ValueError(f"bound array has {a.size} entries, expected {dim}")
# ... 64 lines not shown
        d.pattern_mode = PATTERN_MODES[pattern] if isinstance(pattern, str) else int(pattern)
        d.device = int(device)
        self._tg = None
        if time_grid is not None:
            self._tg = np.ascontiguousarray(time_grid, dtype=np.float64)
            d.time_grid = _dp(self._tg)
            d.time_grid_len = len(self._tg)
            d.grid_size = len(self._tg) - 1
        else:
            d.time_grid = None
            d.time_grid_len = 0
            d.grid_size = int(grid_size)
        if steps is not None:
            d.step_begin, d.step_end = int(steps[0]), int(steps[1])
        d.stream, d.stream_mode = None, 0
        d.control_steps = int(control_steps)
        d.value_order = VALUE_ORDERS[value_order] if isinstance(value_order, str) else int(value_order)
        d.reserved0 = 0
        self.value_order = {0: "csc", 1: "csr"}.get(d.value_order, str(d.value_order))
        self.control_steps = max(1, int(control_steps))
        if int(device) >= 0 and stream != "own":
            if stream == "torch":
                try:
                    import torch
                    if torch.cuda.is_available():
                        d.stream = C.c_void_p(torch.cuda.current_stream(int(device)).cuda_stream)
                        d.stream_mode = 1
                except ImportError:
                    pass
            elif stream is not None:
                d.stream, d.stream_mode = C.c_void_p(int(stream)), 1
        self._stream_raw = int(d.stream or 0) if d.stream_mode == 1 else None
        h = C.c_void_p()
        st = L.ctd_create(C.byref(d), C.byref(h))
        if st != _lib.CTD_OK:
            _raise(st, L.ctd_last_error(None).decode())
        self._h = h
        self.device = int(device)
        self._load_static()
        if d.pattern_mode == 0 and self.dropped_nonzeros() > 0:
            import warnings
            warnings.warn(f"pattern='manual' reproduces the reference's DOCP_Jacobian_pattern, which omits {self.dropped_nonzeros()} "
                          f"structural nonzeros for {self.problem_name} / {self.scheme}; pass pattern='structural' (or 'optimized') "
                          "to solve with a complete Jacobian", stacklevel=2)

    def _load_static(self):
        L = _lib.lib()
        nvar, ncon, nnzj, nnzh = (C.c_int64() for _ in range(4))
        self._ck(L.ctd_sizes(self._h, C.byref(nvar), C.byref(ncon), C.byref(nnzj), C.byref(nnzh)))
        self.dim_NLP_variables, self.dim_NLP_constraints = nvar.value, ncon.value
        self.nnzj, self.nnzh = nnzj.value, nnzh.value
        o = np.zeros(16, dtype=np.int64)
        self._ck(L.ctd_dims(self._h, _ip(o)))
        self.dims = SimpleNamespace(NLP_x=int(o[0]), NLP_u=int(o[1]), NLP_v=int(o[2]), path_cons=int(o[3]),
                                    boundary_cons=int(o[4]))
        self.flags = SimpleNamespace(freet0=bool(o[11]), freetf=bool(o[12]), lagrange=bool(o[13]), mayer=bool(o[14]),
                                     max=bool(o[15]))
        stage = int(o[9])
        self.discretization = SimpleNamespace(_step_variables_block=int(o[6]), _state_stage_eqs_block=int(o[7]),
                                              _step_pathcons_block=int(o[8]), stage=stage, _final_control=bool(o[10]))
        steps = int(o[5])
        nrm = np.zeros(steps + 1)
        fx = np.zeros(steps + 1)
        self._ck(L.ctd_time_grid(self._h, _dp(nrm), _dp(fx)))
        self.time = SimpleNamespace(steps=steps, control_steps=getattr(self, "control_steps", 1), normalized_grid=nrm, fixed_grid=fx)
        if stage > 0:
            a = np.zeros(stage * stage); b = np.zeros(stage); c = np.zeros(stage)
            self._ck(L.ctd_butcher(self._h, _dp(a), _dp(b), _dp(c)))
            self.discretization.butcher_a = a.reshape(stage, stage)
            self.discretization.butcher_b, self.discretization.butcher_c = b, c
        sh = np.zeros(8, dtype=np.int64)
        self._ck(L.ctd_shard_info(self._h, _ip(sh)))
        self.shard = SimpleNamespace(step_begin=int(sh[0]), step_end=int(sh[1]), c_row_begin=int(sh[2]), c_row_end=int(sh[3]),
                                     vals_main_begin=int(sh[4]), vals_main_end=int(sh[5]), owns_first=bool(sh[6]),
                                     owns_last=bool(sh[7]))
        self._bounds = None

    def _ck(self, st):
        if st != _lib.CTD_OK:
            _raise(st, _lib.lib().ctd_last_error(self._h).decode() or _lib.lib().ctd_strerror(st).decode())

    def close(self):
        if getattr(self, "_h", None):
            _lib.lib().ctd_destroy(self._h)
            self._h = None

    def __del__(self):
        try:
            self.close()
        except Exception:
            pass

    @property
    def bounds(self):
        if self._bounds is None:
            lv = np.zeros(self.dim_NLP_variables); uv = np.zeros(self.dim_NLP_variables)
            lc = np.zeros(self.dim_NLP_constraints); uc = np.zeros(self.dim_NLP_constraints)
            self._ck(_lib.lib().ctd_bounds(self._h, _dp(lv), _dp(uv), _dp(lc), _dp(uc)))
            self._bounds = SimpleNamespace(var_l=lv, var_u=uv, con_l=lc, con_u=uc)
        return self._bounds

    def launch_info(self):
        o = np.zeros(8, dtype=np.int64)
        self._ck(_lib.lib().ctd_launch_info(self._h, _ip(o)))
        return dict(grid=int(o[0]), block=int(o[1]), lds_bytes=int(o[2]), steps_per_tile=int(o[3]),
                    csc_period=int(o[4]), edge_entries=int(o[5]), direct_tiles=int(o[6]), workgroups_per_cu=int(o[7]))

    def dropped_nonzeros(self):
        n = C.c_int64()
        self._ck(_lib.lib().ctd_dropped_nonzeros(self._h, C.byref(n)))
        return n.value

    def _check_x(self, x):
        n = x.numel() if _is_tensor(x) else x.size
        if n != self.dim_NLP_variables:
            raise ValueError(f"x has {n} entries, expected dim_NLP_variables = {self.dim_NLP_variables}")

    def _dev_ptr(self, t, n, name):
        import torch
        if not (t.is_cuda and t.dtype == torch.float64 and t.is_contiguous() and t.numel() == n):
            raise ValueError(f"{name} must be a contiguous float64 tensor of {n} entries on the handle's GPU")
        if t.device.index != self.device:
            raise ValueError(f"{name} lives on cuda:{t.device.index}, handle is bound to device {self.device}")
        return C.c_void_p(t.data_ptr())

    def cons_jac(self, x, c=None, vals=None, sync=True):
        L = _lib.lib()
        self._check_x(x)
        if _is_tensor(x):
            import torch
            if c is None:
                c = torch.empty(self.dim_NLP_constraints, dtype=torch.float64, device=x.device)
            if vals is None:
                vals = torch.empty(self.nnzj, dtype=torch.float64, device=x.device)
            fn = L.ctd_cons_jac_dev if sync else L.ctd_cons_jac_dev_async
            self._ck(fn(self._h, self._dev_ptr(x, self.dim_NLP_variables, "x"),
                        self._dev_ptr(c, self.dim_NLP_constraints, "c"), self._dev_ptr(vals, self.nnzj, "vals")))
            return c, vals
        x = np.ascontiguousarray(x, dtype=np.float64)
        c = np.empty(self.dim_NLP_constraints) if c is None else _host_out(c, self.dim_NLP_constraints, "c")
        vals = np.empty(self.nnzj) if vals is None else _host_out(vals, self.nnzj, "vals")
        self._ck(L.ctd_cons_jac(self._h, _dp(x), _dp(c), _dp(vals)))
        return c, vals

    def bind_cons_jac(self, x, c, vals, sync=False):
        L = _lib.lib()
        fn = L.ctd_cons_jac_dev if sync else L.ctd_cons_jac_dev_async
        h = self._h
        px = self._dev_ptr(x, self.dim_NLP_variables, "x")
        pc = self._dev_ptr(c, self.dim_NLP_constraints, "c")
        pv = self._dev_ptr(vals, self.nnzj, "vals")
        ck = self._ck

        def call():
            st = fn(h, px, pc, pv)
            if st:
                ck(st)
        return call

    def set_x_shards(self, step_begins, x_ptrs, self_index):
        L = _lib.lib()
        if step_begins is None:
            self._ck(L.ctd_set_x_shards(self._h, 0, None, None, 0))
            return
        G = len(x_ptrs)
        sb = np.ascontiguousarray(step_begins, dtype=np.int64)
        assert sb.size == G + 1
        arr = (C.c_void_p * G)(*[int(p) if p else None for p in x_ptrs])
        self._ck(L.ctd_set_x_shards(self._h, G, _ip(sb), arr, int(self_index)))

    def stitch_c(self, comm, n_ranks, rank, c):
        self._ck(_lib.lib().ctd_stitch_c(self._h, C.c_void_p(int(comm)), int(n_ranks), int(rank),
                                         self._dev_ptr(c, self.dim_NLP_constraints, "c")))
        return c

    def cons(self, x, c=None):
        L = _lib.lib()
        self._check_x(x)
        if _is_tensor(x):
            import torch
            if c is None:
                c = torch.empty(self.dim_NLP_constraints, dtype=torch.float64, device=x.device)
            self._ck(L.ctd_cons_jac_dev(self._h, self._dev_ptr(x, self.dim_NLP_variables, "x"),
                                        self._dev_ptr(c, self.dim_NLP_constraints, "c"), None))
            return c
        x = np.ascontiguousarray(x, dtype=np.float64)
        c = np.empty(self.dim_NLP_constraints) if c is None else _host_out(c, self.dim_NLP_constraints, "c")
        self._ck(L.ctd_cons(self._h, _dp(x), _dp(c)))
        return c

    def jac_coord(self, x, vals=None):
        L = _lib.lib()
        self._check_x(x)
        if _is_tensor(x):
            import torch
            if vals is None:
                vals = torch.empty(self.nnzj, dtype=torch.float64, device=x.device)
            self._ck(L.ctd_cons_jac_dev(self._h, self._dev_ptr(x, self.dim_NLP_variables, "x"), None,
                                        self._dev_ptr(vals, self.nnzj, "vals")))
            return vals
        x = np.ascontiguousarray(x, dtype=np.float64)
        vals = np.empty(self.nnzj) if vals is None else _host_out(vals, self.nnzj, "vals")
        self._ck(L.ctd_jac_coord(self._h, _dp(x), _dp(vals)))
        return vals

    def obj(self, x):
        L = _lib.lib()
        self._check_x(x)
        f = C.c_double()
        if _is_tensor(x):
            self._ck(L.ctd_obj_dev(self._h, self._dev_ptr(x, self.dim_NLP_variables, "x"), C.byref(f)))
        else:
            x = np.ascontiguousarray(x, dtype=np.float64)
            self._ck(L.ctd_obj(self._h, _dp(x), C.byref(f)))
        return f.value

    def obj_async(self, x, f):
        self._check_x(x)
        self._ck(_lib.lib().ctd_obj_dev_async(self._h, self._dev_ptr(x, self.dim_NLP_variables, "x"), self._dev_ptr(f, 1, "f")))
        return f

    def grad(self, x, g=None, sync=True):
        L = _lib.lib()
        self._check_x(x)
        if _is_tensor(x):
            import torch
            if g is None:
                g = torch.empty(self.dim_NLP_variables, dtype=torch.float64, device=x.device)
            fn = L.ctd_grad_dev if sync else L.ctd_grad_dev_async
            self._ck(fn(self._h, self._dev_ptr(x, self.dim_NLP_variables, "x"), self._dev_ptr(g, self.dim_NLP_variables, "g")))
            return g
        x = np.ascontiguousarray(x, dtype=np.float64)
        g = np.empty(self.dim_NLP_variables) if g is None else _host_out(g, self.dim_NLP_variables, "g")
        self._ck(L.ctd_grad(self._h, _dp(x), _dp(g)))
        return g

    def _prod(self, x, d, out, sync, transpose):
        nin, nout = ((self.dim_NLP_constraints, self.dim_NLP_variables) if transpose
                     else (self.dim_NLP_variables, self.dim_NLP_constraints))
        name = "w" if transpose else "v"
        L = _lib.lib()
# ... 631 lines not shown
```

### include/ctdirect_hip.h

```cpp
#ifndef CTDIRECT_HIP_H
#define CTDIRECT_HIP_H

#include <stddef.h>
#include <stdint.h>

#ifdef __cplusplus
extern "C" {
#endif

typedef struct ctd_handle ctd_handle;

enum {
    CTD_OK = 0,
    CTD_EINVAL = 1,
    CTD_EGRID = 2,
    CTD_ESCHEME = 3,
    CTD_EPATTERN = 4,
    CTD_EPROBLEM = 5,
    CTD_ENODEVICE = 6,
    CTD_EHIP = 7,
    CTD_ENOMEM = 8,
    CTD_ERCCL = 9
};

// ... 36 lines not shown
    int64_t grid_size;
    const double* time_grid;
    int64_t time_grid_len;
    int64_t step_begin;
    int64_t step_end;
    void* stream;
    int32_t stream_mode;
    int32_t control_steps;
    int32_t value_order;
    int32_t reserved0;
} ctd_desc;

enum { CTD_ORDER_CSC = 0, CTD_ORDER_CSR = 1 };

enum { CTD_STREAM_OWN = 0, CTD_STREAM_GIVEN = 1 };

typedef struct ctd_init {
    int32_t use_problem_default;
    const double* state;
    const double* control;
    const double* variable;
    int64_t n_samples;
    const double* t_samples;
    const double* state_samples;
    const double* control_samples;
} ctd_init;

typedef struct ctd_ocp_def {
    const char* name;
    int32_t n, m, nv, npath, nbc;
    int32_t it0, itf;
    double t0, tf;
    int32_t maximize;
    int32_t reserved;
    const char* const* dynamics;
    const char* lagrange;
    const char* mayer;
    const char* const* path;
    const char* const* boundary;
    const char* constants;
    const double *state_lb, *state_ub, *control_lb, *control_ub, *variable_lb, *variable_ub;
    const double *path_lb, *path_ub, *boundary_lb, *boundary_ub;
} ctd_ocp_def;
int32_t ctd_register_ocp(const ctd_ocp_def* def, int32_t* problem_id);
int32_t ctd_ocp_source(int32_t problem_id, char* buf, int64_t cap);
int32_t ctd_jit_check(int32_t problem_id, int32_t scheme);

int32_t ctd_create(const ctd_desc* desc, ctd_handle** out);
int32_t ctd_destroy(ctd_handle* h);
const char* ctd_last_error(const ctd_handle* h);
int32_t ctd_host_alloc(void** ptr, size_t bytes);
int32_t ctd_host_free(void* ptr);
const char* ctd_strerror(int32_t status);

int32_t ctd_sizes(const ctd_handle* h, int64_t* nvar, int64_t* ncon, int64_t* nnzj, int64_t* nnzh);
int32_t ctd_dims(const ctd_handle* h, int64_t* out16);
int32_t ctd_time_grid(const ctd_handle* h, double* normalized, double* fixed);
int32_t ctd_time_grid_at(const ctd_handle* h, const double* x, double* grid);
int32_t ctd_butcher(const ctd_handle* h, double* a, double* b, double* c);
int32_t ctd_bounds(const ctd_handle* h, double* lvar, double* uvar, double* lcon, double* ucon);
int32_t ctd_initial_guess(const ctd_handle* h, double* x0, const ctd_init* init);
int32_t ctd_jac_structure(const ctd_handle* h, int64_t* rows, int64_t* cols);
int32_t ctd_jac_csc(const ctd_handle* h, int64_t* colptr, int64_t* rowval);
int32_t ctd_jac_csr(const ctd_handle* h, int64_t* rowptr, int64_t* colind);
int32_t ctd_value_order(const ctd_handle* h, int32_t* order);
int32_t ctd_dropped_nonzeros(const ctd_handle* h, int64_t* count);

int32_t ctd_obj(ctd_handle* h, const double* x, double* f);
int32_t ctd_grad(ctd_handle* h, const double* x, double* g);
int32_t ctd_cons(ctd_handle* h, const double* x, double* c);
int32_t ctd_jac_coord(ctd_handle* h, const double* x, double* vals);
int32_t ctd_cons_jac(ctd_handle* h, const double* x, double* c, double* vals);

int32_t ctd_cons_jac_dev(ctd_handle* h, const double* x_dev, double* c_dev, double* vals_dev);
int32_t ctd_cons_jac_dev_async(ctd_handle* h, const double* x_dev, double* c_dev, double* vals_dev);
int32_t ctd_obj_dev(ctd_handle* h, const double* x_dev, double* f_host);
int32_t ctd_grad_dev(ctd_handle* h, const double* x_dev, double* g_dev);
int32_t ctd_set_stream(ctd_handle* h, void* stream);
int32_t ctd_obj_dev_async(ctd_handle* h, const double* x_dev, double* f_dev);
int32_t ctd_grad_dev_async(ctd_handle* h, const double* x_dev, double* g_dev);
int32_t ctd_grad_shard_dev_async(ctd_handle* h, const double* x_dev, double* g_dev);
int32_t ctd_sync(ctd_handle* h);

int32_t ctd_shard_info(const ctd_handle* h, int64_t* out8);

int32_t ctd_time_cons_jac_dev(ctd_handle* h, const double* x_dev, double* c_dev, double* vals_dev,
                              int32_t iters, double* mean_ms);
int32_t ctd_debug_stamps(ctd_handle* h, const double* x_dev, double* c_dev, double* vals_dev, uint64_t* out, int64_t cap);
int32_t ctd_launch_info(const ctd_handle* h, int64_t* out8);


int32_t ctd_eval_all_dev_async(ctd_handle* h, const double* x_dev, const double* y_dev, double obj_weight, double* f_dev,
                               double* g_dev, double* c_dev, double* vals_dev, double* hvals_dev);

int32_t ctd_cons_jac_batch_dev_async(ctd_handle* h, int32_t batch, const double* x_dev, int64_t ldx, double* c_dev, int64_t ldc,
                                     double* vals_dev, int64_t ldv);
int32_t ctd_obj_batch_dev_async(ctd_handle* h, int32_t batch, const double* x_dev, int64_t ldx, double* f_dev);
int32_t ctd_grad_batch_dev_async(ctd_handle* h, int32_t batch, const double* x_dev, int64_t ldx, double* g_dev, int64_t ldg);
int32_t ctd_hess_coord_batch_dev_async(ctd_handle* h, int32_t batch, const double* x_dev, int64_t ldx, const double* y_dev, int64_t ldy,
                                       double obj_weight, double* vals_dev, int64_t ldh);

int32_t ctd_jprod(ctd_handle* h, const double* x, const double* v, double* Jv);
int32_t ctd_jtprod(ctd_handle* h, const double* x, const double* w, double* Jtw);
int32_t ctd_jprod_dev_async(ctd_handle* h, const double* x_dev, const double* v_dev, double* Jv_dev);
int32_t ctd_jtprod_dev_async(ctd_handle* h, const double* x_dev, const double* w_dev, double* Jtw_dev);

int32_t ctd_hprod(ctd_handle* h, const double* x, const double* y, double obj_weight, const double* v, double* Hv);
int32_t ctd_hprod_dev_async(ctd_handle* h, const double* x_dev, const double* y_dev, double obj_weight, const double* v_dev,
                            double* Hv_dev);

int32_t ctd_kktprod(ctd_handle* h, const double* x, const double* y, double obj_weight, const double* dx, const double* dy,
                    const double* sx, const double* sc, double* rx, double* rc);
int32_t ctd_kktprod_dev_async(ctd_handle* h, const double* x_dev, const double* y_dev, double obj_weight, const double* dx_dev,
                              const double* dy_dev, const double* sx_dev, const double* sc_dev, double* rx_dev, double* rc_dev);

int32_t ctd_hdiag(ctd_handle* h, const double* x, const double* y, double obj_weight, double* Hd);
int32_t ctd_jsq_rows(ctd_handle* h, const double* x, const double* wx, double* out);
int32_t ctd_jsq_cols(ctd_handle* h, const double* x, const double* wc, double* out);
int32_t ctd_hdiag_dev_async(ctd_handle* h, const double* x_dev, const double* y_dev, double obj_weight, double* Hd_dev);
int32_t ctd_jsq_rows_dev_async(ctd_handle* h, const double* x_dev, const double* wx_dev, double* out_dev);
int32_t ctd_jsq_cols_dev_async(ctd_handle* h, const double* x_dev, const double* wc_dev, double* out_dev);

int32_t ctd_jprod_shard_dev_async(ctd_handle* h, const double* x_dev, const double* v_dev, double* Jv_dev);
int32_t ctd_jtprod_shard_dev_async(ctd_handle* h, const double* x_dev, const double* w_dev, double* Jtw_dev);
int32_t ctd_hprod_shard_dev_async(ctd_handle* h, const double* x_dev, const double* y_dev, double obj_weight, const double* v_dev,
                                  double* Hv_dev);
int32_t ctd_kktprod_shard_dev_async(ctd_handle* h, const double* x_dev, const double* y_dev, double obj_weight, const double* dx_dev,
                                    const double* dy_dev, const double* sx_dev, const double* sc_dev, double* rx_dev, double* rc_dev);

int32_t ctd_hess_structure(const ctd_handle* h, int64_t* rows, int64_t* cols);
int32_t ctd_hess_csc(const ctd_handle* h, int64_t* colptr, int64_t* rowval);
int32_t ctd_hess_csr(const ctd_handle* h, int64_t* rowptr, int64_t* colind);
int32_t ctd_hess_coord(ctd_handle* h, const double* x, const double* y, double obj_weight, double* vals);
int32_t ctd_hess_coord_dev(ctd_handle* h, const double* x_dev, const double* y_dev, double obj_weight, double* vals_dev);
int32_t ctd_hess_coord_dev_async(ctd_handle* h, const double* x_dev, const double* y_dev, double obj_weight, double* vals_dev);
int32_t ctd_time_hess_dev(ctd_handle* h, const double* x_dev, const double* y_dev, double obj_weight, double* vals_dev,
                          int32_t iters, double* mean_ms);
int32_t ctd_hess_launch_info(ctd_handle* h, int64_t* out10);
int32_t ctd_hess_kernel_info(ctd_handle* h, int64_t* out2);
int32_t ctd_hess_shard_info(const ctd_handle* h, int64_t* out13);
int32_t ctd_hess_debug_stamps(ctd_handle* h, const double* x_dev, const double* y_dev, double obj_weight, double* vals_dev,
                              uint64_t* out, int64_t cap);


typedef struct ctd_sharded ctd_sharded;

enum {
    CTD_X_IN_PLACE = 0,
    CTD_X_SHARDED = 1,
    CTD_X_FROM_DEVICE0 = 2,
    CTD_X_SHARDED_COPY = 3,
    CTD_X_SHARDED_IN_PLACE = 4
};

int32_t ctd_create_sharded(const ctd_desc* desc, const int32_t* devices, int32_t n_devices, ctd_sharded** out);
int32_t ctd_sharded_destroy(ctd_sharded* s);
const char* ctd_sharded_last_error(const ctd_sharded* s);
int32_t ctd_sharded_handle(ctd_sharded* s, int32_t k, ctd_handle** h);
int32_t ctd_sharded_shard_info(const ctd_sharded* s, int32_t k, int64_t* out10);
int32_t ctd_cons_jac_sharded_dev_async(ctd_sharded* s, double* const* x_dev, double* const* c_dev, double* const* vals_dev,
                                       int32_t x_mode, int32_t stitch);
int32_t ctd_set_x_shards(ctd_handle* h, int32_t n_shards, const int64_t* step_begin, const double* const* x_bufs, int32_t self);
int32_t ctd_stitch_c(ctd_handle* h, void* nccl_comm, int32_t n_ranks, int32_t rank, double* c_dev);
int32_t ctd_shard_steps(int64_t N, int32_t n_shards, int32_t k, int64_t* begin, int64_t* end);

#define CTD_IPC_HANDLE_BYTES 64
// ... 15 lines not shown
```

Measured before the change: 178,700.

## Skip rewriting constant Jacobian entries on bound cons_jac calls

Adds a binding API that remembers the output buffers for constraint and Jacobian evaluation. After the first full write, later calls launch a SKIPC kernel variant that emits only the Jacobian positions whose values depend on x. The constant positions are classified on the host and uploaded as a compact code and position table. This cuts store traffic and emit work per call, but relies on the caller not overwriting the vals buffer between calls unless it invalidates the binding. It also adds a new kernel instantiation that may change register usage.

```diff
diff --git a/ctdirect.jl_amd/_lib.py b/ctdirect.jl_amd/_lib.py
--- a/ctdirect.jl_amd/_lib.py
+++ b/ctdirect.jl_amd/_lib.py
@@ -63,6 +63,13 @@
     "ctd_cons_jac": (C.c_int32, [_vp, _dp, _dp, _dp]),
     "ctd_cons_jac_dev": (C.c_int32, [_vp, _vp, _vp, _vp]),
     "ctd_cons_jac_dev_async": (C.c_int32, [_vp, _vp, _vp, _vp]),
+    "ctd_jac_const_mask": (C.c_int32, [_vp, C.POINTER(C.c_uint8)]),
+    "ctd_jac_const_info": (C.c_int32, [_vp, _ip]),
+    "ctd_cons_jac_bind": (C.c_int32, [_vp, _vp, _vp, C.POINTER(_vp)]),
+    "ctd_cons_jac_bound_dev": (C.c_int32, [_vp, _vp]),
+    "ctd_cons_jac_bound_dev_async": (C.c_int32, [_vp, _vp]),
+    "ctd_binding_invalidate": (C.c_int32, [_vp]),
+    "ctd_binding_free": (None, [_vp]),
     "ctd_obj_dev": (C.c_int32, [_vp, _vp, _dp]),
     "ctd_obj_dev_async": (C.c_int32, [_vp, _vp, _vp]),
     "ctd_grad_dev_async": (C.c_int32, [_vp, _vp, _vp]),
diff --git a/ctdirect.jl_amd/csrc/ctd_engine.hip b/ctdirect.jl_amd/csrc/ctd_engine.hip
--- a/ctdirect.jl_amd/csrc/ctd_engine.hip
+++ b/ctdirect.jl_amd/csrc/ctd_engine.hip
@@ -2,6 +2,7 @@
 #include <hip/hiprtc.h>
 #include <dlfcn.h>
 
+#include <algorithm>
 #include <cstdio>
 #include <functional>
 #include <map>
@@ -57,6 +58,7 @@
     hipFunction_t f[5] = {};
 };
 
+struct ctd_binding;
 struct ctd_handle {
     Model model;
     int device = -1;
@@ -71,6 +73,9 @@
     DevBuf<double> d_tau;
     DevBuf<uint32_t> d_tmpl, d_vtmpl;
     DevBuf<uint16_t> d_pos;
+    DevBuf<uint32_t> d_skip;
+    int skip_ok = 0;
+    std::vector<ctd_binding*> bindings;
     DevBuf<int64_t> d_edge_idx;
     DevBuf<uint32_t> d_edge_code;
     DevBuf<> d_x, d_c, d_vals;
@@ -110,6 +115,15 @@
     std::string err;
 };
 
+struct ctd_binding {
+    ctd_handle* h;
+    double* c;
+    double* vals;
+    bool have_const;
+    hipStream_t const_stream;
+};
+
+
 constexpr double kWtMB = 64.0;
 constexpr double kHessWtMB = 16.0;
 
@@ -181,6 +195,7 @@
 }
 
 static void destroy_handle(ctd_handle* h) {
+    for (ctd_binding* b : h->bindings) b->h = nullptr;
     DeviceGuard dg;
     if (h->device >= 0) {
         (void)dg.bind(h->device);
@@ -542,6 +557,22 @@
         }
         hp->kp.edge_idx = hp->d_edge_idx.p;
         hp->kp.edge_code = hp->d_edge_code.p;
+        const int bound_skip = env_int("CTD_BOUND_SKIP", 1);
+        if (bound_skip && !hp->rt && hp->lean_ok && hp->kp.n_early == 0 && !debug_stop && mo.n_var > 0 && mo.n_var < mo.Lseg) {
+            bool has_lean = false;
+            for_problem(mo.problem, [&](auto tag) {
+                using P = typename decltype(tag)::type;
+                for_scheme<true>(mo.L, [&](auto t) { has_lean = HasLean<P, t.sc>::value; });
+            });
+            const bool measured_faster = !hp->kp.wt_store && mo.n_var <= hp->block && 4 * mo.n_var <= mo.Lseg;
+            if (has_lean && (bound_skip >= 2 || measured_faster)) {
+                std::vector<uint32_t> tab(mo.var_code);
+                tab.resize((size_t)mo.n_var + ((size_t)mo.n_var + 1) / 2, 0u);
+                std::memcpy(tab.data() + mo.n_var, mo.var_pos.data(), sizeof(uint16_t) * (size_t)mo.n_var);
+                HIP_TRY(nullptr, upload(hp->d_skip, tab));
+                hp->skip_ok = 1;
+            }
+        }
         hp->obj_blocks = 256;
         HIP_TRY(nullptr, hp->d_partial.ensure(hp->obj_blocks));
         HIP_TRY(nullptr, hp->d_obj.ensure(1));
@@ -951,13 +982,19 @@
 };
 
 static int32_t enqueue_cons_jac(ctd_handle* h, const double* x_dev, double* c_dev, double* vals_dev, hipEvent_t te0 = nullptr,
-                                hipEvent_t te1 = nullptr, const Batch* bt = nullptr) {
+                                hipEvent_t te1 = nullptr, const Batch* bt = nullptr, bool skipc = false) {
     const OnDevice on(h);
     if (on.st) return on.st;
     if (!x_dev) return fail(h, CTD_EINVAL, "x is null");
     KParams kp = h->kp;
     kp.c = c_dev;
     kp.vals = vals_dev;
+    if (skipc) {
+        const int nv = h->model.n_var;
+        kp.pos = reinterpret_cast<const uint16_t*>(h->d_skip.p + nv);
+        kp.n_late = nv;
+        kp.div_late = make_fastdiv((uint32_t)nv);
+    }
     hipError_t e = hipErrorInvalidValue;
     if (bt) {
         BatchLd bl{bt->ldx, bt->ldc, bt->ldv};
@@ -980,7 +1017,7 @@
     }
     for_problem(h->model.problem, [&](auto tag) {
         using P = typename decltype(tag)::type;
-        e = launch_cons_jac<P>(kp, x_dev, h->grid, h->block, h->lds_bytes, h->stream, te0, te1, h->lean_ok);
+        e = launch_cons_jac<P>(kp, x_dev, h->grid, h->block, h->lds_bytes, h->stream, te0, te1, h->lean_ok, skipc ? 1 : 0);
     });
     if (e != hipSuccess) return fail(h, CTD_EHIP, std::string("kernel launch: ") + hipGetErrorString(e));
     return CTD_OK;
@@ -988,6 +1025,63 @@
 
 int32_t ctd_cons_jac_dev_async(ctd_handle* h, const double* x_dev, double* c_dev, double* vals_dev) {
     return enqueue_cons_jac(h, x_dev, c_dev, vals_dev);
+}
+
+int32_t ctd_cons_jac_bind(ctd_handle* h, double* c_dev, double* vals_dev, ctd_binding** out) {
+    if (!h || !out) return CTD_EINVAL;
+    *out = nullptr;
+    if (h->device < 0) return fail(h, CTD_ENODEVICE, "ctd_cons_jac_bind: compute call on a host-only handle (device = -1); there is no CPU fallback");
+    ctd_binding* b = new (std::nothrow) ctd_binding{h, c_dev, vals_dev, false, nullptr};
+    if (!b) return fail(h, CTD_ENOMEM, "ctd_cons_jac_bind: out of memory");
+    h->bindings.push_back(b);
+    *out = b;
+    return CTD_OK;
+}
+
+int32_t ctd_cons_jac_bound_dev_async(ctd_binding* b, const double* x_dev) {
+    if (!b || !b->h) return CTD_EINVAL;
+    ctd_handle* h = b->h;
+    const bool skip = b->have_const && h->skip_ok && b->vals && b->const_stream == h->stream;
+    const int32_t st = enqueue_cons_jac(h, x_dev, b->c, b->vals, nullptr, nullptr, nullptr, skip);
+    if (st || skip || !h->skip_ok || !b->vals) return st;
+    hipStreamCaptureStatus cs = hipStreamCaptureStatusNone;
+    if (hipStreamIsCapturing(h->stream, &cs) != hipSuccess) { (void)hipGetLastError(); return CTD_OK; }
+    if (cs == hipStreamCaptureStatusNone) { b->have_const = true; b->const_stream = h->stream; }
+    return CTD_OK;
+}
+
+int32_t ctd_cons_jac_bound_dev(ctd_binding* b, const double* x_dev) {
+    const int32_t st = ctd_cons_jac_bound_dev_async(b, x_dev);
+    if (st) return st;
+    return ctd_sync(b->h);
+}
+
+int32_t ctd_binding_invalidate(ctd_binding* b) {
+    if (!b) return CTD_EINVAL;
+    b->have_const = false;
+    return CTD_OK;
+}
+
+void ctd_binding_free(ctd_binding* b) {
+    if (!b) return;
+    if (b->h) {
+        std::vector<ctd_binding*>& v = b->h->bindings;
+        v.erase(std::remove(v.begin(), v.end(), b), v.end());
+    }
+    delete b;
+}
+
+int32_t ctd_jac_const_mask(const ctd_handle* h, uint8_t* mask) {
+    if (!h || !mask) return CTD_EINVAL;
+    h->model.const_mask(h->step_begin, h->step_end, mask);
+    return CTD_OK;
+}
+
+int32_t ctd_jac_const_info(const ctd_handle* h, int64_t* o) {
+    if (!h || !o) return CTD_EINVAL;
+    const Model& mo = h->model;
+    o[0] = mo.Lseg; o[1] = mo.n_var; o[2] = mo.seg_base; o[3] = mo.reg_first; o[4] = mo.reg_last; o[5] = h->skip_ok;
+    return CTD_OK;
 }
 
 int32_t ctd_set_stream(ctd_handle* h, void* stream) {
diff --git a/ctdirect.jl_amd/csrc/ctd_host.cpp b/ctdirect.jl_amd/csrc/ctd_host.cpp
--- a/ctdirect.jl_amd/csrc/ctd_host.cpp
+++ b/ctdirect.jl_amd/csrc/ctd_host.cpp
@@ -898,6 +898,32 @@
     return ST_OK;
 }
 
+bool Model::const_position(int k) const {
+    const uint32_t c = tmpl[k];
+    const int ci = code_ci(c);
+    if (code_di(c) != 0 || !(ci == C_ZERO || ci == C_ONE || ci == C_NEG1) || code_drec_raw(c) != 0 || code_crec(c) != 0) return false;
+    const int bt = code_beta(c);
+    const int v = (ci == C_ONE ? 1 : (ci == C_NEG1 ? -1 : 0)) + (bt == 0 ? 0 : (bt == 1 ? 1 : -1));
+    return v >= -1 && v <= 1;
+}
+static void classify_const_positions(Model& mo) {
+    mo.var_pos.clear(); mo.var_code.clear();
+    mo.n_var = mo.Lseg;
+    if (mo.Lseg <= 0 || mo.Lseg >= 65536) return;
+    for (int k = 0; k < mo.Lseg; ++k)
+        if (!mo.const_position(k)) { mo.var_pos.push_back((uint16_t)k); mo.var_code.push_back(mo.tmpl[k]); }
+    mo.n_var = (int)mo.var_pos.size();
+}
+void Model::const_mask(int64_t step_begin, int64_t step_end, uint8_t* mask) const {
+    std::memset(mask, 0, (size_t)nnzj);
+    if (n_var >= Lseg) return;
+    const int64_t a = std::max(step_begin, reg_first), b = std::min(step_end, reg_last);
+    for (int64_t i = a; i < b; ++i) {
+        uint8_t* seg = mask + seg_base + (i - reg_first) * (int64_t)Lseg;
+        for (int k = 0; k < Lseg; ++k) seg[k] = const_position(k) ? 1 : 0;
+    }
+}
+
 static void count_dropped(Model& mo) {
     const Layout& L = mo.L;
     const int64_t N = L.N;
@@ -1038,6 +1064,7 @@
     mo.order = d.value_order;
     st = mo.order == 1 ? build_tables_csr(mo, err) : build_tables(mo, err);
     if (st) return st;
+    classify_const_positions(mo);
     count_dropped(mo);
     return build_hess_model(mo, err);
 }
diff --git a/ctdirect.jl_amd/csrc/ctd_host.hpp b/ctdirect.jl_amd/csrc/ctd_host.hpp
--- a/ctdirect.jl_amd/csrc/ctd_host.hpp
+++ b/ctdirect.jl_amd/csrc/ctd_host.hpp
@@ -75,6 +75,11 @@
     int HL = 0, HH = 0;
     std::vector<uint16_t> pos_order;
     int n_late = 0, n_early = 0, c_early = 0, vr_early = 0;
+    std::vector<uint16_t> var_pos;
+    std::vector<uint32_t> var_code;
+    int n_var = 0;
+    bool const_position(int k) const;
+    void const_mask(int64_t step_begin, int64_t step_end, uint8_t* mask) const;
     std::vector<int64_t> edge_idx;
     std::vector<uint32_t> edge_code;
     int edge_split = 0, edge_split2 = 0;
diff --git a/ctdirect.jl_amd/csrc/ctd_kernel_body.hpp b/ctdirect.jl_amd/csrc/ctd_kernel_body.hpp
--- a/ctdirect.jl_amd/csrc/ctd_kernel_body.hpp
+++ b/ctdirect.jl_amd/csrc/ctd_kernel_body.hpp
@@ -1404,7 +1404,7 @@
 #endif
     static constexpr int value = (seg + 255) / 256 < 1 ? 1 : ((seg + 255) / 256 > CTD_PRE_MAX ? CTD_PRE_MAX : (seg + 255) / 256);
 };
-template <class P, int NB = 1, bool LEAN = false>
+template <class P, int NB = 1, bool LEAN = false, bool SKIPC = false>
 CTD_HD EmitPreT<NB> emit_prefetch(const KParams& kp, const BlockCtx& cx, int tid, int nthr) {
     EmitPreT<NB> pre;
     pre.b = 0u;
@@ -1427,7 +1427,11 @@
     }
     const int Ls = kp.Lseg;
     pre.kpos = 0; pre.eb = 0u; pre.ek = 0;
-    if (!LEAN && kp.n_early > 0) {
+    if constexpr (SKIPC) {
+        const int nl = kp.n_late;
+        const int q = nl <= nthr ? tid - (int)fast_div((uint32_t)tid, kp.div_late) * nl : tid;
+        if (q < nl) { pre.kpos = kp.pos[q]; pre.b = skip_codes(kp)[q]; }
+    } else if (!LEAN && kp.n_early > 0) {
         const int q = tid - (int)fast_div((uint32_t)tid, kp.div_late) * kp.n_late;
         pre.kpos = kp.pos[q];
         pre.b = kp.tmpl[pre.kpos];
@@ -1460,7 +1464,7 @@
     return pre;
 }
 
-template <class P, int SC, int S, int NB = 1, bool B = false, bool LEAN = false>
+template <class P, int SC, int S, int NB = 1, bool B = false, bool LEAN = false, bool SKIPC = false>
 CTD_HD void phase_emit_impl(const KParams& kp, const BlockCtx& cx, int tid, int nthr, const EmitPreT<NB> pre_v, const bool hp,
                             const BatchLd bl = BatchLd{}) {
     const Layout& L = kp.L;
@@ -1523,7 +1527,7 @@
             const int nreg = (int)(rb - ra);
             double* out = out_vals<B>(kp, bl) + kp.seg_base + (ra - kp.reg_first) * (int64_t)Ls;
             const int sl0 = (int)(ra - cx.lo);
-            const bool late_only = !LEAN && kp.n_early > 0;
+            const bool late_only = SKIPC || (!LEAN && kp.n_early > 0);
             const int Lw = late_only ? kp.n_late : Ls;
             const int par = (int)fast_div((uint32_t)nthr, late_only ? kp.div_late : kp.div_Lseg);
             if (par >= 1) {
@@ -1550,6 +1554,34 @@
                             if (s < nreg) emit_store(&out[s * Ls + k], a[u] * b[u] + beta, kp.wt_store);
                         }
                     }
+                }
+            } else if constexpr (SKIPC) {
+                const uint32_t* vcodes = skip_codes(kp);
+                uint32_t code = hp ? pre_->b : (tid < Lw ? vcodes[tid] : 0u);
+                int k = hp ? pre_->kpos : (tid < Lw ? (int)kp.pos[tid] : 0);
+                for (int q = tid; q < Lw; q += nthr) {
+                    const bool more = q + nthr < Lw;
+                    const uint32_t nxt = more ? vcodes[q + nthr] : 0u;
+                    const int nk = more ? (int)kp.pos[q + nthr] : 0;
+                    const int bt = code_beta(code);
+                    const double beta = bt == 0 ? 0.0 : (bt == 1 ? 1.0 : -1.0);
+                    const double* pc = cx.rec + (sl0 - code_crec(code)) * stride + R.oC + code_ci(code);
+                    const double* pd = cx.rec + (sl0 - code_drec(code)) * stride + code_di(code);
+                    const int last = nreg - 1;
+                    for (int s0 = 0; s0 < nreg; s0 += 4) {
+                        double a[4], b[4];
+#pragma unroll
+                        for (int u = 0; u < 4; ++u) {
+                            const int s = s0 + u < last ? s0 + u : last;
+                            a[u] = pc[s * stride];
+                            b[u] = pd[s * stride];
+                        }
+#pragma unroll
+                        for (int u = 0; u < 4; ++u)
+                            if (s0 + u < nreg) emit_store(&out[(s0 + u) * Ls + k], a[u] * b[u] + beta, kp.wt_store);
+                    }
+                    code = nxt;
+                    k = nk;
                 }
             } else {
                 uint32_t code = (hp && tid < Ls) ? pre_->b : (tid < Ls ? cx.codes[tid] : 0u);
@@ -1618,11 +1650,11 @@
     }
     CTD_SUBE(kp, 3);
 }
-template <class P, int SC, int S, int NB = 1, bool B = false, bool LEAN = false>
+template <class P, int SC, int S, int NB = 1, bool B = false, bool LEAN = false, bool SKIPC = false>
 CTD_HD void phase_emit(const KParams& kp, const BlockCtx& cx, int tid, int nthr, const EmitPreT<NB>* pre = nullptr,
                        const BatchLd bl = BatchLd{}) {
-    if (pre != nullptr) phase_emit_impl<P, SC, S, NB, B, LEAN>(kp, cx, tid, nthr, *pre, pre->have != 0, bl);
-    else phase_emit_impl<P, SC, S, NB, B, LEAN>(kp, cx, tid, nthr, EmitPreT<NB>{}, false, bl);
+    if (pre != nullptr) phase_emit_impl<P, SC, S, NB, B, LEAN, SKIPC>(kp, cx, tid, nthr, *pre, pre->have != 0, bl);
+    else phase_emit_impl<P, SC, S, NB, B, LEAN, SKIPC>(kp, cx, tid, nthr, EmitPreT<NB>{}, false, bl);
 }
 
 }
diff --git a/ctdirect.jl_amd/csrc/ctd_kernels.hpp b/ctdirect.jl_amd/csrc/ctd_kernels.hpp
--- a/ctdirect.jl_amd/csrc/ctd_kernels.hpp
+++ b/ctdirect.jl_amd/csrc/ctd_kernels.hpp
@@ -27,10 +27,11 @@
     }
 }
 
-template <int S, bool LEAN = false>
+template <int S, bool LEAN = false, bool SKIPC = false>
 __device__ __forceinline__ void ctd_pin_kernargs(const KParams& kp, const double* xu) {
 #if defined(__HIP_DEVICE_COMPILE__)
     if constexpr (LEAN) {
+        if constexpr (SKIPC) asm volatile("" ::"s"(kp.pos), "s"(kp.n_late), "s"(kp.div_late.M), "s"(kp.div_late.d));
         asm volatile("" ::"s"(kp.has_edge), "s"(kp.ntiles), "s"(kp.T), "s"(kp.HL), "s"(kp.HH), "s"(kp.step_begin),
                      "s"(kp.step_end), "s"(kp.L.N), "s"(kp.L.v_off), "s"(kp.L.stagewise), "s"(kp.L.euler), "s"(kp.tau), "s"(kp.L.t0),
                      "s"(kp.L.tf), "s"(xu), "s"(blockDim.x));
@@ -51,10 +52,14 @@
 #endif
 }
 
-template <bool LEAN = false>
+template <bool LEAN = false, bool SKIPC = false>
 __device__ __forceinline__ void ctd_pin_emit_kernargs(const KParams& kp) {
 #if defined(__HIP_DEVICE_COMPILE__)
-    if constexpr (LEAN)
+    if constexpr (LEAN && SKIPC)
+        asm volatile("" ::"s"(kp.c), "s"(kp.vals), "s"(kp.Lseg), "s"(kp.vr), "s"(kp.div_late.M), "s"(kp.div_vr.M),
+                     "s"(kp.div_late.d), "s"(kp.div_vr.d), "s"(kp.seg_base), "s"(kp.reg_first), "s"(kp.reg_last),
+                     "s"(kp.vcol_base[0]), "s"(kp.n_late), "s"(kp.pos));
+    else if constexpr (LEAN)
         asm volatile("" ::"s"(kp.c), "s"(kp.vals), "s"(kp.Lseg), "s"(kp.vr), "s"(kp.div_Lseg.M), "s"(kp.div_vr.M),
                      "s"(kp.div_Lseg.d), "s"(kp.div_vr.d), "s"(kp.seg_base), "s"(kp.reg_first), "s"(kp.reg_last),
                      "s"(kp.vcol_base[0]));
@@ -65,25 +70,25 @@
 #endif
 }
 
-template <class P, int SC, int S, bool DBG, bool B = false, bool LEAN = false>
+template <class P, int SC, int S, bool DBG, bool B = false, bool LEAN = false, bool SKIPC = false>
 __device__ __forceinline__ void cons_jac_body(const KParams& kp, const double* __restrict__ xu, int block, double* ctd_lds,
                                               const BatchLd bl = BatchLd{}) {
     if constexpr (B) xu += batch_member() * bl.ldx;
-    ctd_pin_kernargs<SC == SC_IRK ? S : 0, LEAN>(kp, xu);
+    ctd_pin_kernargs<SC == SC_IRK ? S : 0, LEAN, SKIPC>(kp, xu);
     ctd_stamp<DBG>(kp, 0);
     if (DBG && kp.debug_stop == 1) return;
     const int tid = (int)threadIdx.x, nthr = (int)blockDim.x;
     if constexpr (DirectTile<P, SC>::value) {
         const BlockCtx cx = make_direct_ctx<LEAN>(kp, block, ctd_lds, xu, LV<P, SC, S, LEAN>::blk(kp), LEAN ? P::NV : -1);
-        const EmitPre pre = emit_prefetch<P, 1, LEAN>(kp, cx, tid, nthr);
+        const EmitPre pre = emit_prefetch<P, 1, LEAN, SKIPC>(kp, cx, tid, nthr);
         ctd_stamp<DBG>(kp, 1);
         phase_eval<P, SC, S, RegEval<P, SC, S>::value, 1, B, LEAN>(kp, cx, tid, nthr, &pre, bl);
-        ctd_pin_emit_kernargs<LEAN>(kp);
+        ctd_pin_emit_kernargs<LEAN, SKIPC>(kp);
         __syncthreads();
         ctd_stamp<DBG>(kp, 2);
         ctd_stamp<DBG>(kp, 3);
         if (DBG && kp.debug_stop >= 2 && kp.debug_stop <= 4) return;
-        phase_emit<P, SC, S, 1, B, LEAN>(kp, cx, tid, nthr, &pre, bl);
+        phase_emit<P, SC, S, 1, B, LEAN, SKIPC>(kp, cx, tid, nthr, &pre, bl);
         ctd_stamp<DBG>(kp, 4);
         if (DBG && kp.stamps) {
             __builtin_amdgcn_s_waitcnt(0);
@@ -95,8 +100,8 @@
     BlockCtx cx = make_ctx<LEAN>(kp, block, ctd_lds);
     constexpr int NB = EmitN<P, SC, S>::value;
     EmitPreT<NB> pre = {};
-    const bool use_pre = !cx.is_edge && !codes_staged(kp);
-    if (use_pre) pre = emit_prefetch<P, NB, LEAN>(kp, cx, tid, nthr);
+    const bool use_pre = !cx.is_edge && (SKIPC || !codes_staged(kp));
+    if (use_pre) pre = emit_prefetch<P, NB, LEAN, SKIPC>(kp, cx, tid, nthr);
     phase_load<P, SC, S, true, LEAN>(kp, cx, xu, tid, nthr);
     const int nblk = kp.ntiles + kp.has_edge;
     for (;;) {
@@ -104,7 +109,7 @@
         ctd_stamp<DBG>(kp, 1);
         if (DBG && kp.debug_stop == 2) return;
         phase_eval<P, SC, S, false, 1, B, LEAN>(kp, cx, tid, nthr, nullptr, bl);
-        ctd_pin_emit_kernargs<LEAN>(kp);
+        ctd_pin_emit_kernargs<LEAN, SKIPC>(kp);
         __syncthreads();
         ctd_stamp<DBG>(kp, 2);
         if (DBG && kp.debug_stop == 3) return;
@@ -126,7 +131,7 @@
             nx = make_ctx<LEAN>(kp, block, ctd_lds);
             tin = load_issue<P>(kp, nx, xu, tid, nthr);
         }
-        phase_emit_impl<P, SC, S, NB, B, LEAN>(kp, cx, tid, nthr, pre, use_pre, bl);
+        phase_emit_impl<P, SC, S, NB, B, LEAN, SKIPC>(kp, cx, tid, nthr, pre, use_pre, bl);
         ctd_stamp<DBG>(kp, 4);
         if (!more) break;
         load_commit<P, SC, S>(kp, nx, xu, tin, tid, nthr);
@@ -143,10 +148,10 @@
     static constexpr int value = (P::NX <= 12 && !(SC == SC_MIDPOINT && S > 1)) ? 4 : 1;
 };
 
-template <class P, int SC, int S, bool DBG, bool LEAN = false>
+template <class P, int SC, int S, bool DBG, bool LEAN = false, bool SKIPC = false>
 __global__ void __launch_bounds__(P::MAXB, (MinWaves<P, SC, S>::value)) cons_jac_kernel(const KParams kp, const double* __restrict__ xu) {
     extern __shared__ double ctd_lds[];
-    cons_jac_body<P, SC, S, DBG, false, LEAN>(kp, xu, (int)blockIdx.x, ctd_lds);
+    cons_jac_body<P, SC, S, DBG, false, LEAN, SKIPC>(kp, xu, (int)blockIdx.x, ctd_lds);
 }
 template <class P, int SC, int S>
 __global__ void __launch_bounds__(P::MAXB, (MinWaves<P, SC, S>::value)) cons_jac_batch_kernel(const KParams kp, const double* __restrict__ xu,
@@ -616,25 +621,27 @@
 #endif
 
 #if !defined(__HIPCC_RTC__)
-template <class P, int SC, int S, bool DBG, bool LEAN>
+template <class P, int SC, int S, bool DBG, bool LEAN, bool SKIPC = false>
 hipError_t launch_variant_dbg(const KParams& kp, const double* xu, int grid, int block, size_t lds_bytes, hipStream_t st,
                               hipEvent_t e0, hipEvent_t e1) {
     if (lds_bytes > 64 * 1024) {
-        hipError_t e = hipFuncSetAttribute((const void*)cons_jac_kernel<P, SC, S, DBG, LEAN>, hipFuncAttributeMaxDynamicSharedMemorySize,
+        hipError_t e = hipFuncSetAttribute((const void*)cons_jac_kernel<P, SC, S, DBG, LEAN, SKIPC>, hipFuncAttributeMaxDynamicSharedMemorySize,
                                            (int)lds_bytes);
         if (e != hipSuccess) return e;
     }
-    if (e0 || e1) hipExtLaunchKernelGGL((cons_jac_kernel<P, SC, S, DBG, LEAN>), dim3(grid), dim3(block), lds_bytes, st, e0, e1, 0, kp, xu);
-    else cons_jac_kernel<P, SC, S, DBG, LEAN><<<grid, block, lds_bytes, st>>>(kp, xu);
+    if (e0 || e1) hipExtLaunchKernelGGL((cons_jac_kernel<P, SC, S, DBG, LEAN, SKIPC>), dim3(grid), dim3(block), lds_bytes, st, e0, e1, 0, kp, xu);
+    else cons_jac_kernel<P, SC, S, DBG, LEAN, SKIPC><<<grid, block, lds_bytes, st>>>(kp, xu);
     return hipGetLastError();
 }
+template <class P, int SC> struct HasLean { static constexpr bool value = DirectTile<P, SC>::value || SC == SC_IRK; };
 template <class P, int SC, int S>
 hipError_t launch_variant(const KParams& kp, const double* xu, int grid, int block, size_t lds_bytes, hipStream_t st,
-                          hipEvent_t e0, hipEvent_t e1, int lean_ok) {
+                          hipEvent_t e0, hipEvent_t e1, int lean_ok, int skipc) {
     const bool dbg = kp.stamps || kp.debug_stop;
-    constexpr bool kHasLean = DirectTile<P, SC>::value || SC == SC_IRK;
+    constexpr bool kHasLean = HasLean<P, SC>::value;
     if constexpr (kHasLean) {
         if (lean_ok && kp.halo == nullptr && kp.n_early == 0) {
+            if (skipc && !dbg) return launch_variant_dbg<P, SC, S, false, true, true>(kp, xu, grid, block, lds_bytes, st, e0, e1);
             if (dbg) return launch_variant_dbg<P, SC, S, true, true>(kp, xu, grid, block, lds_bytes, st, e0, e1);
             return launch_variant_dbg<P, SC, S, false, true>(kp, xu, grid, block, lds_bytes, st, e0, e1);
         }
@@ -645,9 +652,9 @@
 
 template <class P>
 hipError_t launch_cons_jac(const KParams& kp, const double* xu, int grid, int block, size_t lds_bytes, hipStream_t st,
-                           hipEvent_t e0, hipEvent_t e1, int lean_ok) {
+                           hipEvent_t e0, hipEvent_t e1, int lean_ok, int skipc) {
     hipError_t e = hipErrorInvalidValue;
-    for_scheme<true>(kp.L, [&](auto t) { e = launch_variant<P, t.sc, t.s>(kp, xu, grid, block, lds_bytes, st, e0, e1, lean_ok); });
+    for_scheme<true>(kp.L, [&](auto t) { e = launch_variant<P, t.sc, t.s>(kp, xu, grid, block, lds_bytes, st, e0, e1, lean_ok, skipc); });
     return e;
 }
 
@@ -696,14 +703,14 @@
 
 #define CTD_INSTANTIATE_LAUNCHERS(P)                                                                                       \
     template hipError_t launch_cons_jac<P>(const KParams&, const double*, int, int, size_t, hipStream_t, hipEvent_t, \
-                                           hipEvent_t, int);                                                                 \
+                                           hipEvent_t, int, int);                                                            \
     template hipError_t launch_cons_jac_batch<P>(const KParams&, const double*, const BatchLd&, int, int, size_t, hipStream_t, int); \
     template hipError_t launch_obj<P>(const ObjParams&, const double*, int, int, hipStream_t, int);                  \
     template int occupancy_cons_jac<P>(const KParams&, int, size_t);                                                 \
     template hipError_t launch_grad<P>(const GradParams&, const double*, int, hipStream_t, int);
 #define CTD_EXTERN_LAUNCHERS(P)                                                                                            \
     extern template hipError_t launch_cons_jac<P>(const KParams&, const double*, int, int, size_t, hipStream_t,      \
-                                                  hipEvent_t, hipEvent_t, int);                                              \
+                                                  hipEvent_t, hipEvent_t, int, int);                                         \
     extern template hipError_t launch_cons_jac_batch<P>(const KParams&, const double*, const BatchLd&, int, int, size_t, hipStream_t, \
                                                         int);                                                                      \
     extern template hipError_t launch_obj<P>(const ObjParams&, const double*, int, int, hipStream_t, int);          \
diff --git a/ctdirect.jl_amd/csrc/ctd_layout.hpp b/ctdirect.jl_amd/csrc/ctd_layout.hpp
--- a/ctdirect.jl_amd/csrc/ctd_layout.hpp
+++ b/ctdirect.jl_amd/csrc/ctd_layout.hpp
@@ -211,6 +211,7 @@
     int32_t wg_stride;
     int32_t wt_store;
 };
+CTD_HD const uint32_t* skip_codes(const KParams& kp) { return reinterpret_cast<const uint32_t*>(kp.pos) - kp.n_late; }
 struct BatchLd {
     int64_t ldx, ldc, ldv;
 };
diff --git a/ctdirect.jl_amd/docp.py b/ctdirect.jl_amd/docp.py
--- a/ctdirect.jl_amd/docp.py
+++ b/ctdirect.jl_amd/docp.py
@@ -1,4 +1,5 @@
 import ctypes as C
+import os
 from types import SimpleNamespace
 
 import numpy as np
@@ -229,6 +230,9 @@
 
     def close(self):
         if getattr(self, "_h", None):
+            for f in getattr(self, "_bindings", ()):
+                f()
+            self._bindings = []
             _lib.lib().ctd_destroy(self._h)
             self._h = None
 
@@ -291,19 +295,47 @@
         return c, vals
 
     def bind_cons_jac(self, x, c, vals, sync=False):
-        L = _lib.lib()
-        fn = L.ctd_cons_jac_dev if sync else L.ctd_cons_jac_dev_async
-        h = self._h
+        import weakref
+        L = _lib.lib()
         px = self._dev_ptr(x, self.dim_NLP_variables, "x")
         pc = self._dev_ptr(c, self.dim_NLP_constraints, "c")
         pv = self._dev_ptr(vals, self.nnzj, "vals")
         ck = self._ck
+        if os.environ.get("CTD_LIB_PATH") and not hasattr(L, "ctd_cons_jac_bind"):
+            h, full = self._h, (L.ctd_cons_jac_dev if sync else L.ctd_cons_jac_dev_async)
+
+            def call_full():
+                st = full(h, px, pc, pv)
+                if st:
+                    ck(st)
+            call_full.invalidate = call_full.close = lambda: None
+            return call_full
+        fn = L.ctd_cons_jac_bound_dev if sync else L.ctd_cons_jac_bound_dev_async
+        b = C.c_void_p()
+        ck(L.ctd_cons_jac_bind(self._h, pc, pv, C.byref(b)))
 
         def call():
-            st = fn(h, px, pc, pv)
+            st = fn(b, px)
             if st:
                 ck(st)
+
+        def invalidate():
+            ck(L.ctd_binding_invalidate(b))
+        call.invalidate = invalidate
+        call.close = weakref.finalize(call, L.ctd_binding_free, b)
+        self._bindings = [f for f in getattr(self, "_bindings", ()) if f.alive] + [call.close]
         return call
+
+    def jac_const_mask(self):
+        mask = np.zeros(self.nnzj, dtype=np.uint8)
+        self._ck(_lib.lib().ctd_jac_const_mask(self._h, mask.ctypes.data_as(C.POINTER(C.c_uint8))))
+        return mask
+
+    def jac_const_info(self):
+        o = np.zeros(6, dtype=np.int64)
+        self._ck(_lib.lib().ctd_jac_const_info(self._h, _ip(o)))
+        return dict(period=int(o[0]), variable=int(o[1]), seg_base=int(o[2]), reg_first=int(o[3]), reg_last=int(o[4]),
+                    bound_skips=bool(o[5]))
 
     def set_x_shards(self, step_begins, x_ptrs, self_index):
         L = _lib.lib()
diff --git a/include/ctdirect_hip.h b/include/ctdirect_hip.h
--- a/include/ctdirect_hip.h
+++ b/include/ctdirect_hip.h
@@ -142,6 +142,15 @@
 int32_t ctd_grad_shard_dev_async(ctd_handle* h, const double* x_dev, double* g_dev);
 int32_t ctd_sync(ctd_handle* h);
 
+typedef struct ctd_binding ctd_binding;
+int32_t ctd_cons_jac_bind(ctd_handle* h, double* c_dev, double* vals_dev, ctd_binding** out);
+int32_t ctd_cons_jac_bound_dev_async(ctd_binding* b, const double* x_dev);
+int32_t ctd_cons_jac_bound_dev(ctd_binding* b, const double* x_dev);
+int32_t ctd_binding_invalidate(ctd_binding* b);
+void ctd_binding_free(ctd_binding* b);
+int32_t ctd_jac_const_mask(const ctd_handle* h, uint8_t* mask);
+int32_t ctd_jac_const_info(const ctd_handle* h, int64_t* out6);
+
 int32_t ctd_shard_info(const ctd_handle* h, int64_t* out8);
 
 int32_t ctd_time_cons_jac_dev(ctd_handle* h, const double* x_dev, double* c_dev, double* vals_dev,
diff --git a/profiles/cons_jac_resources.py b/profiles/cons_jac_resources.py
--- /dev/null
+++ b/profiles/cons_jac_resources.py
@@ -0,0 +1,75 @@
+import argparse
+import os
+import re
+import subprocess
+import tempfile
+from concurrent.futures import ThreadPoolExecutor
+
+ROOT = os.path.dirname(os.path.dirname(os.path.abspath(__file__)))
+CSRC = os.path.join(ROOT, "ctdirect.jl_amd", "csrc")
+HIPCC = os.environ.get("HIPCC", "/opt/rocm/bin/hipcc")
+SCHEMES = {(0, 1): "trapeze", (1, 1): "midpoint / Euler", (1, 2): "midpoint, 2 controls", (1, 3): "midpoint, 3 controls",
+           (2, 1): "Gauss-Legendre 1", (2, 2): "Gauss-Legendre 2", (2, 3): "Gauss-Legendre 3"}
+VARIANTS = {(0, 0): "general", (1, 0): "lean", (1, 1): "lean+SKIPC"}
+
+
+def kernels(stem):
+    with tempfile.TemporaryDirectory() as tmp:
+        asm = os.path.join(tmp, stem + ".s")
+        r = subprocess.run([HIPCC, "--offload-arch=gfx950", "-O3", "-std=c++17", "-fPIC", "-ffp-contract=off", "--cuda-device-only",
+                            "-S", f"ctd_kern_{stem}.hip", "-o", asm], cwd=CSRC, capture_output=True, text=True)
+        if r.returncode:
+            raise SystemExit(r.stderr[-4000:])
+        with open(asm) as f:
+            text = f.read()
+    meta = {}
+    for m in re.finditer(r"\.amdhsa_kernel (\S+)(.*?)\.end_amdhsa_kernel", text, re.S):
+        g = lambda k: int(re.search(k + r" (\d+)", m.group(2)).group(1))
+        meta[m.group(1)] = (g(r"\.amdhsa_next_free_sgpr"), g(r"\.amdhsa_next_free_vgpr"), g(r"\.amdhsa_private_segment_fixed_size"))
+    out = []
+    for m in re.finditer(r"^(_ZN3ctd15cons_jac_kernelINS_\d+(\w+?)ELi(\d+)ELi(\d+)((?:ELb\d)+)EEEv\S*):[^\n]*\n(.*?)^\.Lfunc_end", text, re.S | re.M):
+        name, prob, sc, s, flags, body = m.group(1), m.group(2), int(m.group(3)), int(m.group(4)), re.findall(r"ELb(\d)", m.group(5)), m.group(6)
+        dbg, lean, skipc = (int(f) for f in (flags + ["0", "0"])[:3])
+        if dbg:
+            continue
+        ins = [l for l in body.splitlines() if re.match(r"\s+[a-z]\w*", l) and not l.lstrip().startswith((".", ";"))]
+        rounds, pending = 0, False
+        for l in ins:
+            if re.match(r"\s+s_load", l):
+                pending = True
+            elif "s_waitcnt" in l and "lgkmcnt(0)" in l and pending:
+                rounds, pending = rounds + 1, False
+        sg, vg, scratch = meta[name]
+        out.append((prob, sc, s, VARIANTS[(lean, skipc)],
+                    dict(sgpr=sg, vgpr=vg, scratch=scratch, wl=sum("v_writelane" in l for l in ins), rl=sum("v_readlane" in l for l in ins),
+                         s_load=sum(bool(re.match(r"\s+s_load", l)) for l in ins), rounds=rounds, instr=len(ins))))
+    return sorted(out, key=lambda k: (k[1], k[2], list(VARIANTS.values()).index(k[3])))
+
+
+def main():
+    ap = argparse.ArgumentParser()
+    ap.add_argument("--jobs", type=int, default=4)
+    ap.add_argument("problems", nargs="*", default=["goddard", "double_integrator_path", "quadrotor", "quadrotor12"])
+    args = ap.parse_args()
+    with ThreadPoolExecutor(args.jobs) as ex:
+        table = list(ex.map(kernels, args.problems))
+    lines = ["# python profiles/cons_jac_resources.py: cons_jac_kernel<OCP, scheme class, stages, false, LEAN, SKIPC>, compiler figures\n",
+             "# (next_free_sgpr does not count the 6 of VCC / flat scratch / XNACK that profiles/lean_kernel.md includes)\n"]
+    bad = []
+    for rows in table:
+        lean = {(p, sc, s): f for p, sc, s, v, f in rows if v == "lean"}
+        for p, sc, s, v, f in rows:
+            lines.append(f"{p} {SCHEMES.get((sc, s), (sc, s))} {v}: sgpr={f['sgpr']} vgpr={f['vgpr']} scratch={f['scratch']} lane_spills={f['wl']}/{f['rl']} "
+                         f"s_load={f['s_load']} rounds={f['rounds']} instructions={f['instr']}\n")
+            if v == "lean+SKIPC" and (f["vgpr"] > 128 or (f["scratch"] > 0 and lean[(p, sc, s)]["scratch"] == 0)):
+                bad.append(lines[-1])
+    path = os.path.join(ROOT, "profiles", "cons_jac_resource_usage.log")
+    with open(path, "w") as f:
+        f.writelines(lines)
+    print(path, len(lines) - 2, "kernels")
+    if bad:
+        raise SystemExit("SKIPC instantiations over budget:\n" + "".join(bad))
+
+
+if __name__ == "__main__":
+    main()
```

Measured after the change: 176,800. -1.1%, worse.
